# schulter/crbm

Measured on AMD Instinct MI355X. Metric: Gibbs-steps/sec (PCD-1) at batch 8192x4x200, 10 motifs len 15, higher is better.
Workload: dtype f32; 1 GPU; cfg2: 10 motifs len 15, batch 8192 x 4x200, PCD-1, single-stranded; chains_per_gpu=8192, gibbs_steps_per_launch=1, visible=4x200, hidden=10x186, parallelism=chains sharded over 1 GPU(s), no collective in the Gibbs step

## Files before the change

### __graft_entry__.py

```python
import os
import sys

ROOT = os.path.dirname(os.path.abspath(__file__))
if ROOT not in sys.path:
    sys.path.insert(0, ROOT)


PRECOMPILE = [dict(num_motifs=k, motif_length=m, doublestranded=ds) for (k, m, ds) in [
    (10, 15, 0), (10, 15, 1), (50, 25, 0), (20, 15, 1),
    (10, 5, 1), (10, 5, 0), (3, 4, 1), (4, 5, 1), (4, 5, 0), (6, 9, 1), (2, 5, 1),
]]
PRECOMPILE += [dict(num_motifs=6, motif_length=7, doublestranded=1, pooling=2, fantasy_hidden_len=24),
               dict(num_motifs=10, motif_length=15, doublestranded=0, pooling=4, fantasy_hidden_len=48),
               dict(num_motifs=5, motif_length=8, doublestranded=1, pooling=3, fantasy_hidden_len=36)]
PRECOMPILE += [dict(num_motifs=100, motif_length=15, doublestranded=0), dict(num_motifs=20, motif_length=40, doublestranded=1)]
PRECOMPILE += [dict(num_motifs=300, motif_length=10, doublestranded=0, fantasy_hidden_len=51), dict(num_motifs=120, motif_length=40, doublestranded=1, fantasy_hidden_len=61),
               dict(num_motifs=256, motif_length=4, doublestranded=1, fantasy_hidden_len=37), dict(num_motifs=300, motif_length=10, doublestranded=0, batchsize=4096, fantasy_hidden_len=191)]
PRECOMPILE += [dict(num_motifs=300, motif_length=10, doublestranded=0, batchsize=512, fantasy_hidden_len=30),
               dict(num_motifs=120, motif_length=40, doublestranded=1, batchsize=256, fantasy_hidden_len=24)]
PRECOMPILE += [dict(num_motifs=10, motif_length=15, doublestranded=0, batchsize=8192, fantasy_hidden_len=186),
               dict(num_motifs=50, motif_length=25, doublestranded=0, batchsize=8192, fantasy_hidden_len=976),
               dict(num_motifs=20, motif_length=15, doublestranded=1, batchsize=8192, fantasy_hidden_len=486)]
PRECOMPILE += [dict(num_motifs=3, motif_length=3, doublestranded=1, batchsize=4, fantasy_hidden_len=8),
               dict(num_motifs=4, motif_length=4, doublestranded=0, batchsize=4, fantasy_hidden_len=8)]

STATISTICS_SHAPES = [dict(num_motifs=k, motif_length=m, doublestranded=ds, pooling=pool, batchsize=7, fantasy_hidden_len=lf)
                     for (k, m, ds, pool, lf) in [
    (10, 15, 0, 1, 33), (16, 16, 1, 1, 33), (16, 32, 0, 1, 33), (32, 16, 0, 1, 33), (8, 12, 1, 1, 33), (20, 15, 1, 1, 33),
    (33, 17, 0, 1, 33), (64, 32, 1, 1, 33), (20, 40, 1, 1, 33), (4, 64, 1, 1, 33), (100, 15, 0, 1, 33), (130, 7, 1, 1, 33),
    (256, 4, 0, 1, 33), (6, 7, 1, 2, 34), (10, 15, 0, 4, 36), (5, 8, 1, 3, 33), (300, 10, 0, 1, 33), (150, 6, 1, 2, 34),
    (10, 15, 0, 1, 64), (10, 15, 0, 1, 32), (20, 40, 1, 1, 64), (20, 40, 1, 1, 32)]]


def build():
    from crbm_amd.csrc import build as hip_build
    hip_build.build(verbose=True)
    hip_build.prune_cache()
    hip_build.precompile(PRECOMPILE + STATISTICS_SHAPES, verbose=False)
    from oracle import build_cpu
    build_cpu.build(verbose=True)
    import crbm_amd
    from crbm_amd import _lib
    lib = _lib.load()
    assert lib.crbm_abi_version() == _lib.ABI_VERSION
    print("crbm_amd", crbm_amd.__version__, "ABI", lib.crbm_abi_version())


def smoke():
    import numpy as np
    from crbm_amd import CRBM
    from oracle.crbm_oracle import OracleCRBM, synthetic_onehot

    K, M, B, Lf, n, L = 10, 15, 64, 186, 48, 200
    W = np.random.default_rng(42).standard_normal((K, 1, 4, M)).astype(np.float32)
    model = CRBM(K, M, doublestranded=False, batchsize=B, cd_k=1, fantasy_hidden_len=Lf, seed=2026)
    oracle = OracleCRBM(K, M, doublestranded=False, batchsize=B, cd_k=1, fantasy_hidden_len=Lf, seed=2026, W=W)
    b = (oracle.b + 4.0).astype(np.float32)
    model.motifs.set_value(W)
    model.bias.set_value(b)
    oracle.b = b.astype(np.float64)
    D = synthetic_onehot(n, L, seed=1234)
    model._trainingFct(D)
    oracle.train_step(D)
    np.testing.assert_allclose(model.motifs.get_value(), oracle.W, rtol=1e-4, atol=2e-6)
    np.testing.assert_allclose(model.bias.get_value(), oracle.b, rtol=1e-4, atol=2e-6)
    np.testing.assert_allclose(model.c.get_value(), oracle.c, rtol=1e-4, atol=2e-6)
    from oracle.crbm_oracle import hidden_uniforms, visible_uniforms, KIND_CHAIN_H, KIND_CHAIN_V
    model.set_fantasy(oracle.fantasy_h.astype(np.float32))
    idx = np.arange(B) + oracle.seq_offset
    for _ in range(3):
        t = oracle.gibbs_step
        model.set_rng(gibbs_step=t)
        uv = visible_uniforms(oracle.seed, t, idx, Lf + M - 1, KIND_CHAIN_V)
        Pv, v = oracle._computeVgivenH(oracle.fantasy_h, None, uv)
        uh = hidden_uniforms(oracle.seed, t, idx, K, Lf, 0, KIND_CHAIN_H)
        P, hnew = oracle._computeHgivenV(v, False, uh)
        model.gibbsSteps(1)
        h, _ = model.get_fantasy()
        gv = model.get_fantasy_visible()
        badv = (gv != v).any(axis=2)[:, 0]
        if badv.any():
            gap = np.min(np.abs(np.cumsum(Pv[:, 0], axis=1)[:, :3] - uv[:, None, :]), axis=1)
            assert np.all(gap[badv] < 1e-6), "visible sample differs away from a tie"
        bad = (h != hnew) & ~badv.any(axis=1)[:, None, None, None]
        assert np.all(np.abs(P - uh)[bad] < 1e-6), "hidden sample differs away from a tie"
        oracle.fantasy_h, oracle.gibbs_step = hnew, t + 1
        model.set_fantasy(hnew.astype(np.float32))
    assert oracle.fantasy_h.sum() > 0
    np.testing.assert_allclose(model.freeEnergy(D), oracle.freeEnergy(D), rtol=1e-4)
    print("smoke ok: train step, Gibbs chain and free energy match the oracle")


if __name__ == "__main__":
    build()
    if os.path.exists("/dev/kfd"):
        smoke()
```

### crbm_amd/_lib.py

```python
import ctypes
import os

import numpy as np

_HERE = os.path.dirname(os.path.abspath(__file__))
LIB_PATH = os.path.join(_HERE, "csrc", "libcrbm_hip.so")

UNIQUE_ID_BYTES = 128
IPC_HANDLE_BYTES = 64
ABI_VERSION = 5

CRBM_OK = 0
ERR_INVALID, ERR_HIP, ERR_NOT_ONEHOT, ERR_NOT_BINARY, ERR_RCCL, ERR_NO_GPU, ERR_IPC_TIMEOUT = -1, -2, -3, -4, -5, -6, -7


class CrbmConfig(ctypes.Structure):
    _fields_ = [
        ("num_motifs", ctypes.c_int32),
        ("motif_length", ctypes.c_int32),
        ("input_dims", ctypes.c_int32),
        ("doublestranded", ctypes.c_int32),
        ("batchsize", ctypes.c_int32),
        ("cd_k", ctypes.c_int32),
        ("pooling", ctypes.c_int32),
# ... 25 lines not shown
_I32P = ctypes.POINTER(ctypes.c_int32)
_I64P = ctypes.POINTER(ctypes.c_int64)


class CrbmSite(ctypes.Structure):
    _fields_ = [("seq", ctypes.c_int32), ("motif", ctypes.c_int32), ("start", ctypes.c_int32),
                ("strand", ctypes.c_int32), ("prob", ctypes.c_float)]


_SITEP = ctypes.POINTER(CrbmSite)
_SITES_TAIL = [ctypes.c_float, _I64, _SITEP, _I64P, _I32P, _I32P, _F]

SIGNATURES = {
    "crbm_create": (_I32, [ctypes.POINTER(CrbmConfig), ctypes.POINTER(_H)]),
    "crbm_precompile": (_I32, [ctypes.POINTER(CrbmConfig)]),
    "crbm_destroy": (_I32, [_H]),
    "crbm_last_error": (ctypes.c_char_p, [_H]),
    "crbm_abi_version": (_I32, []),
    "crbm_device_count": (_I32, []),
    "crbm_set_params": (_I32, [_H, _F, _F, _F]),
    "crbm_get_params": (_I32, [_H, _F, _F, _F]),
    "crbm_set_velocities": (_I32, [_H, _F, _F, _F]),
    "crbm_get_velocities": (_I32, [_H, _F, _F, _F]),
    "crbm_set_fantasy": (_I32, [_H, _F, _F]),
    "crbm_get_fantasy": (_I32, [_H, _F, _F]),
    "crbm_get_fantasy_visible": (_I32, [_H, _F]),
    "crbm_set_rng": (_I32, [_H, _U64, _U32, _U32]),
    "crbm_get_rng": (_I32, [_H, ctypes.POINTER(_U64), ctypes.POINTER(_U32), ctypes.POINTER(_U32)]),
    "crbm_set_shard": (_I32, [_H, _U32]),
    "crbm_train_step": (_I32, [_H, _F, _I32, _I32]),
    "crbm_dataset_upload": (_I32, [_H, _F, _I32, _I32]),
    "crbm_dataset_upload_codes": (_I32, [_H, _U8P, _I32, _I32]),
    "crbm_dataset_select": (_I32, [_H, _I32]),
    "crbm_train_step_resident": (_I32, [_H, _I32, _I32]),
    "crbm_train_epoch_resident": (_I32, [_H, _I32]),
    "crbm_train_epoch_sharded": (_I32, [_H, _I32, _I32, _I32]),
    "crbm_gibbs_steps": (_I32, [_H, _I32]),
    "crbm_gibbs_steps_async": (_I32, [_H, _I32]),
    "crbm_sync": (_I32, [_H]),
    "crbm_wait_idle": (_I32, [_H]),
    "crbm_time_gibbs": (_I32, [_H, _I32, _I32, _F]),
    "crbm_time_train": (_I32, [_H, _I32, _I32, _I32, _F]),
    "crbm_h_given_v": (_I32, [_H, _F, _I32, _I32, _I32, _U32, _F, _F, _F]),
    "crbm_v_given_h": (_I32, [_H, _F, _F, _I32, _I32, _U32, _F, _F, _F]),
    "crbm_hit_probs": (_I32, [_H, _F, _I32, _I32, _F]),
    "crbm_free_energy": (_I32, [_H, _F, _I32, _I32, _F]),
    "crbm_free_energy_per_motif": (_I32, [_H, _F, _I32, _I32, _F]),
    "crbm_eval_data": (_I32, [_H, _F, _I32, _I32, _F, _F]),
    "crbm_eval_params": (_I32, [_H, _F, _F, _F]),
    "crbm_hit_probs_codes": (_I32, [_H, _U8P, _I32, _I32, _F]),
    "crbm_hit_probs_resident": (_I32, [_H, _I32, _I32, _F]),
    "crbm_free_energy_codes": (_I32, [_H, _U8P, _I32, _I32, _F, _F]),
    "crbm_free_energy_resident": (_I32, [_H, _I32, _I32, _F, _F]),
    "crbm_eval_data_resident": (_I32, [_H, _I32, _I32, _F, _F]),
    "crbm_eval_epoch_resident": (_I32, [_H, _I32, ctypes.POINTER(ctypes.c_double), ctypes.POINTER(ctypes.c_double)]),
    "crbm_hit_summary": (_I32, [_H, _F, _I32, _I32, _F, _F, _F]),
    "crbm_hit_summary_codes": (_I32, [_H, _U8P, _I32, _I32, _F, _F, _F]),
    "crbm_hit_summary_resident": (_I32, [_H, _I32, _I32, _F, _F, _F]),
    "crbm_motif_sites": (_I32, [_H, _F, _I32, _I32] + _SITES_TAIL),
    "crbm_motif_sites_codes": (_I32, [_H, _U8P, _I32, _I32] + _SITES_TAIL),
    "crbm_motif_sites_resident": (_I32, [_H, _I32, _I32] + _SITES_TAIL),
    "crbm_scan_sites_codes": (_I32, [_H, _U8P, _I64, ctypes.c_float, _I64, _SITEP, _I64P]),
    "crbm_scan_histogram_codes": (_I32, [_H, _U8P, _I64, ctypes.c_float, ctypes.c_float, _I32, ctypes.POINTER(_U64), _I64P]),
    "crbm_variant_effects_codes": (_I32, [_H, _U8P, _I64, _I64, _I64P, _U8P, _F, _F, _I32P]),
    "crbm_mutagenesis": (_I32, [_H, _F, _I32, _I32, _F, _F]),
    "crbm_mutagenesis_codes": (_I32, [_H, _U8P, _I32, _I32, _F, _F]),
    "crbm_mutagenesis_resident": (_I32, [_H, _I32, _I32, _F, _F]),
    "crbm_ais": (_I32, [_H, _I32, _I32, _U32, _F, _I32, _I32, _I32, _F, _U64, _U8P, _F]),
    "crbm_comm_unique_id": (_I32, [_U8P]),
    "crbm_comm_init": (_I32, [_H, _U8P, _I32, _I32]),
    "crbm_comm_destroy": (_I32, [_H]),
    "crbm_comm_broadcast_state": (_I32, [_H, _I32]),
    "crbm_ipc_export": (_I32, [_H, _U8P]),
    "crbm_ipc_attach": (_I32, [_H, _U8P, _I32, _I32]),
    "crbm_ipc_detach": (_I32, [_H]),
    "crbm_ipc_status": (_I32, [_H, ctypes.POINTER(_I32)]),
    "crbm_sums_count": (_I32, [_H]),
    "crbm_train_local": (_I32, [_H, _F, _I32, _I32, _F]),
    "crbm_train_apply": (_I32, [_H, _F, _I32]),
    "crbm_time_allreduce": (_I32, [_H, _I32, _F]),
    "crbm_get_launch_info": (_I32, [_H, ctypes.POINTER(CrbmLaunchInfo)]),
    "crbm_copy_bandwidth": (_I32, [_H, ctypes.c_int64, _I32, _F]),
    "crbm_last_shader_clock": (_I32, [_H, _F]),
    "crbm_gibbs_state_bytes": (ctypes.c_int64, [_H]),
}

_lib = None


class CrbmLibraryError(RuntimeError):
    pass


def load():
    global _lib
    if _lib is not None:
        return _lib
    if not os.path.exists(LIB_PATH):
        raise CrbmLibraryError(
            "HIP extension not built: %s is missing. Run `python -m crbm_amd.csrc.build` "
            "(or __graft_entry__.build()). There is no CPU fallback." % LIB_PATH)
    lib = ctypes.CDLL(LIB_PATH)
    for name, (res, args) in SIGNATURES.items():
        fn = getattr(lib, name)
        fn.restype = res
        fn.argtypes = args
    if lib.crbm_abi_version() != ABI_VERSION:
        raise CrbmLibraryError("ABI version mismatch")
    _lib = lib
    return lib


def fptr(arr):
    if arr is None:
        return None
    assert arr.dtype == np.float32 and arr.flags["C_CONTIGUOUS"]
    return arr.ctypes.data_as(_F)


def as_f32(x):
    return np.ascontiguousarray(x, dtype=np.float32)
```

### crbm_amd/csrc/build.py

```python
import os
import subprocess
import sys
from concurrent.futures import ThreadPoolExecutor

HERE = os.path.dirname(os.path.abspath(__file__))
OBJ = os.path.join(HERE, "build")
LIB = os.path.join(HERE, "libcrbm_hip.so")
HIPCC = os.environ.get("HIPCC", "/opt/rocm/bin/hipcc")
ARCH = "gfx950"
FLAGS = ["--offload-arch=" + ARCH, "-O3", "-std=c++17", "-fPIC", "-ffp-contract=off",
         "-Wall", "-Wno-unused-function", "-Wno-unused-result"]
HEADERS = ["crbm_kernels.h", "crbm_kernels_generic.h", "crbm_layout.h", "crbm_jit.h", "crbm_plan.h", "crbm_sweep.h", os.path.join("..", "..", "include", "crbm_amd.h")]


def _newer(target, deps):
    if not os.path.exists(target):
        return True
    t = os.path.getmtime(target)
    return any(os.path.getmtime(d) > t for d in deps)


def _compile(job):
    src, obj, extra = job
    deps = [os.path.join(HERE, src), os.path.abspath(__file__)] + [os.path.join(HERE, h) for h in HEADERS]
    if not _newer(obj, deps):
        return obj, False
    cmd = [HIPCC] + FLAGS + extra + ["-c", os.path.join(HERE, src), "-o", obj]
    r = subprocess.run(cmd, capture_output=True, text=True)
    if r.returncode != 0:
        raise RuntimeError("hipcc failed: %s\n%s\n%s" % (" ".join(cmd), r.stdout, r.stderr))
    if r.stderr.strip():
        sys.stderr.write(r.stderr)
    return obj, True


def build(verbose=True, jobs=None):
    os.makedirs(OBJ, exist_ok=True)
    work = [("crbm_api.hip", os.path.join(OBJ, "crbm_api.o"), [])]
    jobs = jobs or min(8, os.cpu_count() or 4)
    with ThreadPoolExecutor(max_workers=jobs) as ex:
        results = list(ex.map(_compile, work))
    objs = [o for o, _ in results]
    if any(changed for _, changed in results) or _newer(LIB, objs):
        cmd = [HIPCC, "--offload-arch=" + ARCH, "-shared", "-fPIC", "-o", LIB] + objs + ["-L/opt/rocm/lib", "-lhiprtc", "-ldl"]
        r = subprocess.run(cmd, capture_output=True, text=True)
        if r.returncode != 0:
            raise RuntimeError("link failed: %s\n%s\n%s" % (" ".join(cmd), r.stdout, r.stderr))
        if verbose:
            print("built", LIB)
    elif verbose:
        print("up to date:", LIB)
    return LIB


def prune_cache(verbose=True):
    cache = os.path.join(HERE, "jit_cache")
    if not os.path.isdir(cache):
        return 0
    newest = max(os.path.getmtime(os.path.join(HERE, h)) for h in ("crbm_kernels.h", "crbm_layout.h", "crbm_jit.h"))
    gone = 0
    for f in os.listdir(cache):
        path = os.path.join(cache, f)
        if f.endswith((".hsaco", ".tmp")) and os.path.getmtime(path) < newest:
            os.unlink(path)
            gone += 1
    if verbose and gone:
        print("jit cache: removed %d stale code objects" % gone)
    return gone


def precompile(configs, verbose=True):
    import ctypes
    sys.path.insert(0, os.path.dirname(os.path.dirname(HERE)))
    from crbm_amd import _lib
    lib = _lib.load()
    for c in configs:
        cfg = _lib.CrbmConfig(num_motifs=c["num_motifs"], motif_length=c["motif_length"], input_dims=4,
                              doublestranded=int(c.get("doublestranded", 0)), batchsize=c.get("batchsize", 20),
                              cd_k=1, pooling=c.get("pooling", 1), fantasy_hidden_len=c.get("fantasy_hidden_len", 200),
                              learning_rate=0.1, momentum=0.9, rho=0.01, lambda_rate=0.1, seed=0, device=0, reserved=0)
        rc = lib.crbm_precompile(ctypes.byref(cfg))
        if rc != 0:
            raise RuntimeError("precompile failed for %s: %s" % (c, lib.crbm_last_error(None).decode()))
        if verbose:
            print("jit cache ready:", c)


if __name__ == "__main__":
    build()
```

### crbm_amd/csrc/crbm_api.hip

```cpp
#define CRBM_DEFINE_MISC_KERNELS
#include "crbm_kernels.h"
#include "crbm_jit.h"
#include "crbm_plan.h"
#include "crbm_sweep.h"
#include "../../include/crbm_amd.h"

#include <dlfcn.h>
#include <rccl/rccl.h>

#include <algorithm>
#include <chrono>
#include <condition_variable>
#include <deque>
#include <mutex>
#include <thread>
#include <climits>
#include <cmath>
#include <cstdio>
#include <cstdlib>
#include <cstring>
#include <string>
#include <vector>

using namespace crbm;
// ... 91 lines not shown
};

struct crbm_handle {
  crbm_config cfg;
  int K = 0, M = 0, ds = 0, NW = 0, KAM = 0;
  int A = 4;
  int Lf = 0, Lv = 0, B = 0;
  int device = 0, num_cu = 256;
  hipStream_t stream = nullptr;
  hipStream_t stream2 = nullptr;
  hipEvent_t ev0 = nullptr, ev1 = nullptr, ev_fork = nullptr, ev_join = nullptr;
  bool overlap = false;
  LaunchPlan plan;
  bool big() const { return plan.big; }
  const ModelShape& ms() const { return plan.ms; }
  JitKernels jk;
  float* d_tables = nullptr;
  float* d_tf_solo = nullptr;
  bool tables_dirty = true;
  uint64_t params_version = 1, tf_solo_version = 0;
  float *dW = nullptr, *db = nullptr, *dc = nullptr, *dvW = nullptr, *dvb = nullptr, *dvc = nullptr;
  float *dW2 = nullptr, *db2 = nullptr, *dc2 = nullptr, *dvW2 = nullptr, *dvb2 = nullptr, *dvc2 = nullptr;
  uint32_t *d_hm = nullptr, *d_hmp = nullptr, *d_vf = nullptr;
  uint32_t* d_flags = nullptr;
  unsigned long long* d_ones = nullptr;
  DevBuf<float> stage, stage2, out_a, out_b, out_c;
  DevBuf<uint32_t> letters, letters2, masks_tmp;
  DevBuf<float> out_a2, out_b2;
  DevBuf<uint32_t> dataset[CRBM_DATASET_SLOTS];
  DevBuf<float> partials, partials2;
  DevBuf<unsigned long long> eval_ones;
  struct SetBufs {
    DevBuf<SiteRec> site_recs;
    DevBuf<unsigned long long> site_count, site_keys;
    DevBuf<float> mut_df, mut_pll;
    DevBuf<uint32_t> mut_rows;
    DevBuf<unsigned long long> scan_valid, scan_off;
    DevBuf<unsigned short> scan_lanes;
    DevBuf<uint32_t> scan_tiles;
    DevBuf<int32_t> var_windows;
  } set_bufs[2];
  int mut_route = 0;
  DevBuf<float> ais_betas, ais_base, ais_logw;
  DevBuf<uint8_t> ais_state;
  DevBuf<unsigned long long> hist;
  float* d_sums = nullptr;
  int dataset_n[CRBM_DATASET_SLOTS] = {0, 0}, dataset_L[CRBM_DATASET_SLOTS] = {0, 0};
  int slot = 0;
  uint64_t seed = 0;
  uint32_t gibbs_step = 0, eval_step = 0, chain_offset = 0;
  int LWs = 0;
  hipStream_t part_stream[4] = {nullptr, nullptr, nullptr, nullptr};
  PartWorker* part_worker[4] = {nullptr, nullptr, nullptr, nullptr};
  hipEvent_t part_done[4] = {nullptr, nullptr, nullptr, nullptr};
  hipEvent_t ev_parts_fork = nullptr;
  bool forked = false;
  bool main_idle_hint = false;
  double part_launch_us = 0.0;
  hipEvent_t ev_cal0 = nullptr, ev_cal1 = nullptr;
  bool cal_pending = false;
  int wall_khz = 100000;
  int variant = 1;
  int topdown_mode = 0;
  uint32_t* d_nset = nullptr;
  int nset_slots = 0;
  uint32_t launches_since_read = 0;
  double activity = -1.0;
  int stats_rows = 0;
  bool fuse_stats = false;
  bool one_launch = true;
  SumsLayout sl;
  ncclComm_t comm = nullptr;
  int nranks = 1, rank = 0;
  float* ipc_buf = nullptr;
  void* ipc_peer[IPC_MAX_RANKS] = {};
  int ipc_stride = 0;
  bool ipc_on = false;
  uint32_t ipc_step = 0;
  bool ipc_published = false;
  uint32_t* d_ticket = nullptr;
  unsigned long long* d_probe = nullptr;
  unsigned long long probe_base[2] = {0, 0}, probe_last[2] = {0, 0};
  bool probe_on = false;
  unsigned long long* d_timeline = nullptr;
  int timeline_cap = 0, timeline_next = 0;
  unsigned long long ipc_timeout_ticks = 0;
  SlabModel slab;
  float* d_slab_tables = nullptr;
  int slab_n = 0;
  bool slab_hgv = false;
  uint64_t slab_tables_version = 0;
  std::string slab_note;
  std::string err;
};

namespace {

int fail(crbm_handle* h, int code, const std::string& msg) {
  if (h) h->err = msg; else g_create_error = msg;
  return code;
}

#define HIPCHK(expr)                                                                         \
  do {                                                                                       \
    hipError_t e__ = (expr);                                                                 \
    if (e__ != hipSuccess)                                                                   \
      return fail(h, CRBM_ERR_HIP, std::string(#expr) + ": " + hipGetErrorString(e__));      \
  } while (0)

#define ARGCHK(cond, msg)                                 \
  do {                                                    \
    if (!(cond)) return fail(h, CRBM_ERR_INVALID, msg);   \
  } while (0)

RngView rng_view(const crbm_handle* h, uint32_t step, uint32_t seq_offset) {
  RngView r;
  r.seed_lo = (uint32_t)(h->seed & 0xffffffffu);
  r.seed_hi = (uint32_t)(h->seed >> 32);
  r.step = step;
  r.seq_offset = seq_offset;
  return r;
}

int tab_bytes(const ModelShape& ms) { return ms.TAB * 4; }

int lw(const crbm_handle* h, int L) { return letter_words_any(h->A, L); }

int ensure_tables(crbm_handle* h) {
  if (!h->tables_dirty || h->big()) return CRBM_OK;
  TablesArgs t;
  t.W = h->dW; t.b = h->db; t.c = h->dc; t.out = h->d_tables;
  const unsigned grid = (unsigned)std::max(1, std::min((h->ms().TABLES_ALL + 255) / 256, h->num_cu * 4));
  HIPCHK(jit_launch(h->jk.build_tables, t, grid, 1, 256, 0, h->stream));
  h->tables_dirty = false;
  h->main_idle_hint = false;
  return CRBM_OK;
}

int ensure_solo_table(crbm_handle* h) {
  if (h->plan.GS == h->plan.G || h->tf_solo_version == h->params_version) return CRBM_OK;
  TablesArgs t;
  t.W = h->dW; t.b = h->db; t.c = h->dc; t.out = h->d_tf_solo;
  const unsigned grid = (unsigned)std::max(1, std::min((h->plan.ms_solo.TAB + 255) / 256, h->num_cu * 4));
  HIPCHK(jit_launch(h->jk.build_gather_solo, t, grid, 1, 256, 0, h->stream));
  h->tf_solo_version = h->params_version;
  h->main_idle_hint = false;
  return CRBM_OK;
}

BigModel big_model(const crbm_handle* h) {
  BigModel m;
  m.W = h->dW; m.b = h->db; m.c = h->dc;
  m.K = h->K; m.M = h->M; m.ds = h->ds; m.NW = h->NW; m.A = h->A;
  return m;
}

constexpr int SLAB_FALLBACK = -1000;
bool slab_fe_on(const crbm_handle* h) { return h->slab.K && tab_bytes(h->slab.ms) <= 160 * 1024 && env_int("CRBM_SLAB_FE", 1) != 0; }
int slab_launch_hgv(crbm_handle* h, const uint32_t* d_letters, int n, int L, int mode, unsigned long long* ones, uint32_t* masks,
                    uint32_t kind, uint32_t step, uint32_t seq_offset, hipStream_t st);
int slab_launch_stats(crbm_handle* h, const uint32_t* d_letters, int n, int L, bool data_half, hipStream_t st, ReduceArgs* reduce);
int slab_launch_fe(crbm_handle* h, const uint32_t* rows, int n, int L, float* fe, float* fem, DevBuf<float>* scratch, hipStream_t st);

int big_launch_hgv(crbm_handle* h, const uint32_t* d_letters, int n, int L, int mode, float* act, float* prob, float* sample,
                   unsigned long long* ones, uint32_t* masks, uint32_t kind, uint32_t step, uint32_t seq_offset, hipStream_t st) {
  if (h->slab.K && h->slab_hgv && (masks || ones) && !act && !prob && !sample) {
// ... 78 lines not shown
  BigStatsArgs a;
  a.m = big_model(h);
  a.letters = d_letters;
  a.n = n; a.L = L; a.Lh = L - M + 1; a.LW = lw(h, L);
  a.want_sparsity = data_half ? 1 : 0;
  a.R = std::max(1, std::min(n, std::max(1, (h->num_cu * 8) / K)));
  a.pool = h->ms().POOL;
  a.CH = std::max(64, std::min(4096, a.Lh));
  a.CH = std::max(a.pool, a.CH - a.CH % a.pool);
  a.row = 3 * KAM + 3 * K + h->A;
  a.off_vh0 = 0; a.off_vh1 = KAM; a.off_h0 = 2 * KAM; a.off_h1 = 2 * KAM + K;
  a.off_sw = 2 * KAM + 2 * K; a.off_sb = 3 * KAM + 2 * K; a.off_v = 3 * KAM + 3 * K;
  HIPCHK(pbuf.ensure((size_t)a.R * a.row));
  a.partials = pbuf.p;
  ARGCHK(h->A * M <= BIG_ST * 256, "motif_length too large for the statistics kernel");
  const size_t lds = (((size_t)h->A * M + 3) & ~(size_t)3) * 4 + (size_t)(a.pool > 1 ? 5 : 3) * a.CH * 4 + 64 + 12 * 256 * 4 +
                     (size_t)((h->A + 3) & ~3) * 4 + (size_t)a.CH + M;
  ARGCHK(lds <= 160 * 1024, "motif_length too large for the statistics kernel");
  hipLaunchKernelGGL(big_stats_kernel, dim3(K, a.R), dim3(256), lds, st, a);
  HIPCHK(hipGetLastError());
  *reduce = reduce_args(h, data_half, pbuf.p, a.R, a.row, n);
  return CRBM_OK;
}

int big_launch_eval(crbm_handle* h, const uint32_t* rows, int n, int L, int hits, float* fe, float* fem, float* hmax, float* hmean,
                    unsigned long long* pos_fx, DevBuf<float>* fe_scratch, hipStream_t st) {
  if (!hits && slab_fe_on(h)) {
    const int rc = slab_launch_fe(h, rows, n, L, fe, fem, fe_scratch, st);
    if (rc != SLAB_FALLBACK) return rc;
  }
  BigEvalArgs a;
  a.m = big_model(h);
  a.letters = rows;
  a.n = n; a.L = L; a.Lh = L - h->M + 1; a.LW = lw(h, L);
  a.fe = fe; a.fem = fem; a.hmax = hmax; a.hmean = hmean; a.pos_fx = pos_fx; a.hits = hits; a.pool = h->ms().POOL;
  const size_t lds = (((size_t)h->A * h->M + 3) & ~(size_t)3) * 4 + 64 + (size_t)L;
  ARGCHK(lds <= 160 * 1024, "sequence too long for the evaluation kernel of a model of this size");
  hipLaunchKernelGGL(big_eval_kernel, dim3(std::max(1, std::min(n, h->num_cu * 8))), dim3(256), lds, st, a);
  HIPCHK(hipGetLastError());
  return CRBM_OK;
}

int grid_for(long items, int threads, int cap) {
  long g = (items + threads - 1) / threads;
  return (int)std::max<long>(1, std::min<long>(g, cap));
}

int tile_seqs(int len, int target) { return std::max(1, std::min(target / std::max(1, len), (1 << 20) / std::max(1, len))); }

int check_flags(crbm_handle* h) {
  uint32_t flags = 0;
  HIPCHK(hipMemcpyAsync(&flags, h->d_flags, sizeof(flags), hipMemcpyDeviceToHost, h->stream));
  HIPCHK(hipStreamSynchronize(h->stream));
  if (flags) {
    HIPCHK(hipMemsetAsync(h->d_flags, 0, sizeof(uint32_t), h->stream));
    if (flags & 1u) return fail(h, CRBM_ERR_NOT_ONEHOT, "visible data is not exactly one-hot");
    return fail(h, CRBM_ERR_NOT_BINARY, "hidden state is not exactly 0/1");
  }
  return CRBM_OK;
}

int launch_hgv(crbm_handle* h, const uint32_t* d_letters, int n, int L, int mode, float* act, float* prob,
               float* sample, unsigned long long* ones, uint32_t kind, uint32_t step, uint32_t seq_offset) {
  if (h->big()) return big_launch_hgv(h, d_letters, n, L, mode, act, prob, sample, ones, nullptr, kind, step, seq_offset, h->stream);
  int rc = ensure_tables(h);
  if (rc) return rc;
  HgvArgs a;
  a.tables = h->d_tables;
  a.letters = d_letters;
  a.n = n; a.L = L; a.Lh = L - h->M + 1; a.LW = lw(h, L);
  a.TS = tile_seqs(a.Lh, 4096);
  a.divLh = make_fastdiv((uint32_t)a.Lh);
  a.mode = mode;
  a.act = act; a.prob = prob; a.sample = sample; a.ones = ones;
  a.rng = rng_view(h, step, seq_offset);
  a.kind = kind;
  const int ntiles = (n + a.TS - 1) / a.TS;
  const unsigned gx = (unsigned)std::max(1, std::min(ntiles, h->num_cu * 8));
  HIPCHK(jit_launch(h->jk.hgv, a, gx, 1, 256, (unsigned)tab_bytes(h->ms()), h->stream));
  return CRBM_OK;
}

StatsGeom stats_geom(const StatsMfmaLayout& st, float* partials, long ngroups, int lds_bytes);

int prepare_gibbs(crbm_handle* h, const ChainGeom& g, int steps, ReduceArgs* model_reduce, GibbsArgs* out, unsigned* lds_out) {
  const GibbsLayout& gl = g.gl;
  GibbsArgs& a = *out;
  a.tables = h->d_tables;
  a.tables_tf = nullptr; a.off_ws = 0;
  a.hm = h->d_hm; a.hmp = h->ds ? h->d_hmp : nullptr; a.vout = h->d_vf;
  a.nchains = h->B; a.Lf = h->Lf; a.Lv = gl.Lv; a.S = gl.S;
  a.nvb = gl.nvb; a.nhb = gl.nhb; a.Lrow = gl.Lrow; a.LWs = gl.LWs;
  a.divVB = make_fastdiv((uint32_t)a.nvb);
  a.divHB = make_fastdiv((uint32_t)a.nhb);
  a.divRow = make_fastdiv((uint32_t)(a.Lrow * h->NW));
  a.divLfw = make_fastdiv((uint32_t)(a.Lf * h->NW));
  a.steps = steps;
  a.rng = rng_view(h, h->gibbs_step, h->chain_offset);
  a.ones = h->d_nset;
  a.clock = h->probe_on ? h->d_probe : nullptr;
  a.timeline = nullptr;
  a.debug = env_int("CRBM_GIBBS_DEBUG", 0);
  a.nblocks = g.grid;
  a.stats_off = 0;
  a.sg = StatsGeom();
  unsigned lds = (unsigned)gl.lds_bytes;
  if (model_reduce) {
    const StatsMfmaLayout st = stats_mfma_layout(h->ms(), 0, h->Lf, g.threads, 0, false);
    HIPCHK(h->partials2.ensure((size_t)g.grid * st.row));
    a.stats_off = (gl.lds_bytes / 4 + 3) & ~3;
    lds = (unsigned)std::max((a.stats_off + st.region_floats) * 4, st.combine_bytes);
    a.sg = stats_geom(st, h->partials2.p, (long)gl.S * st.GPC, (int)lds);
    *model_reduce = reduce_args(h, false, h->partials2.p, g.grid, st.row, h->B);
  }
  *lds_out = lds;
  return CRBM_OK;
}

void part_worker_main(PartWorker* w) {
  (void)hipSetDevice(w->device);
  std::unique_lock<std::mutex> lock(w->mu);
  for (;;) {
    const auto spin_until_t = std::chrono::steady_clock::now() + std::chrono::milliseconds(2);
    while (!w->stop && w->jobs.empty() && std::chrono::steady_clock::now() < spin_until_t) {
      lock.unlock();
      for (int i = 0; i < 64; ++i) __builtin_ia32_pause();
      lock.lock();
    }
    w->cv.wait(lock, [&] { return w->stop || !w->jobs.empty(); });
    if (w->jobs.empty()) return;
    PartJob job = w->jobs.front();
    w->jobs.pop_front();
    w->busy = true;
    lock.unlock();
    hipError_t e = hipSuccess;
    if (job.delay_ticks > 0) {
      hipLaunchKernelGGL(delay_kernel, dim3(1), dim3(64), 0, w->stream, job.delay_ticks);
      e = hipGetLastError();
    }
    if (e == hipSuccess) e = jit_launch(job.fn, job.args, job.grid, 1, job.threads, job.lds, w->stream);
    lock.lock();
    if (e != hipSuccess && w->error == hipSuccess) w->error = e;
    w->busy = false;
    if (w->jobs.empty()) w->idle_cv.notify_all();
  }
}

int drain_part_workers(crbm_handle* h) {
  for (int p = 1; p < h->plan.chain_parts; ++p) {
    PartWorker* w = h->part_worker[p];
    if (!w) continue;
    std::unique_lock<std::mutex> lock(w->mu);
    w->idle_cv.wait(lock, [&] { return w->jobs.empty() && !w->busy; });
    if (w->error != hipSuccess) {
      const hipError_t e = w->error;
      w->error = hipSuccess;
      return fail(h, CRBM_ERR_HIP, std::string("chain launch of partition ") + std::to_string(p) + ": " + hipGetErrorString(e));
    }
  }
  return CRBM_OK;
}

int join_parts(crbm_handle* h) {
  if (!h->forked) return CRBM_OK;
  {
    const int rc = drain_part_workers(h);
    if (rc) return rc;
  }
  for (int p = 1; p < h->plan.chain_parts; ++p) {
    HIPCHK(hipEventRecord(h->part_done[p], h->part_stream[p]));
    HIPCHK(hipStreamWaitEvent(h->stream, h->part_done[p], 0));
  }
  h->forked = false;
  return CRBM_OK;
}

int launch_gibbs_parts(crbm_handle* h, int steps) {
  bool first_of_fork = false;
  double stagger_ticks = 0.0;
  if (!h->forked) {
    if (!h->main_idle_hint && hipStreamQuery(h->stream) != hipSuccess) {
      (void)hipGetLastError();
      HIPCHK(hipEventRecord(h->ev_parts_fork, h->stream));
      for (int p = 1; p < h->plan.chain_parts; ++p) HIPCHK(hipStreamWaitEvent(h->part_stream[p], h->ev_parts_fork, 0));
    }
    h->main_idle_hint = false;
    h->forked = true;
    first_of_fork = true;
    if (h->cal_pending && hipEventQuery(h->ev_cal1) == hipSuccess) {
      float ms = 0.f;
      if (hipEventElapsedTime(&ms, h->ev_cal0, h->ev_cal1) == hipSuccess && ms > 0.f) h->part_launch_us = 1e3 * ms;
      h->cal_pending = false;
    }
    (void)hipGetLastError();
    if (env_int("CRBM_PART_STAGGER", 1)) {
      const double est = h->part_launch_us > 0.0 ? h->part_launch_us
                                                 : 1e-3 * (double)h->B * h->Lf * h->K * (1 + h->ds) * steps;
      stagger_ticks = 0.9 * est / h->plan.chain_parts * (h->wall_khz / 1000.0);
    }
  }
  const LaunchPlan& plan = h->plan;
  GibbsArgs a;
  unsigned lds = 0;
  const int rc = prepare_gibbs(h, plan.part, steps, nullptr, &a, &lds);
  if (rc) return rc;
  const unsigned grid = (unsigned)plan.part.grid, threads = (unsigned)plan.part.threads;
  const size_t per = (size_t)h->Lf * h->NW;
  const int waves = (int)threads / 64;
  h->nset_slots = plan.chain_parts * (int)grid * waves;
  for (int p = 0; p < plan.chain_parts; ++p) {
    const int c0 = p * plan.part_chains, n = std::min(plan.part_chains, h->B - c0);
    if (n <= 0) break;
    GibbsArgs ap = a;
    ap.hm = a.hm + (size_t)c0 * per;
    if (ap.hmp) ap.hmp = a.hmp + (size_t)c0 * per;
    ap.vout = a.vout + (size_t)c0 * a.LWs;
    ap.nchains = n;
    ap.rng.seq_offset = a.rng.seq_offset + (uint32_t)c0;
    ap.ones = a.ones + (size_t)p * grid * waves;
    if (p > 0) ap.clock = nullptr;
    if (h->d_timeline && h->timeline_next < h->timeline_cap) ap.timeline = h->d_timeline + 2 * (size_t)(h->timeline_next++);
    ap.nblocks = (int)grid;
    if (p > 0) {
      PartWorker* w = h->part_worker[p];
      {
        std::lock_guard<std::mutex> lock(w->mu);
        w->jobs.push_back(PartJob{h->jk.gibbs_sparse, ap, grid, threads, lds, (unsigned long long)(stagger_ticks * p)});
      }
      w->cv.notify_one();
      continue;
    }
    const bool calibrate = first_of_fork && !h->cal_pending;
    if (calibrate) HIPCHK(hipEventRecord(h->ev_cal0, h->part_stream[0]));
    HIPCHK(jit_launch(h->jk.gibbs_sparse, ap, grid, 1, threads, lds, h->part_stream[0]));
    if (calibrate) {
      HIPCHK(hipEventRecord(h->ev_cal1, h->part_stream[0]));
      h->cal_pending = true;
    }
  }
  h->gibbs_step += (uint32_t)steps;
  h->launches_since_read += 1;
  return CRBM_OK;
}

int launch_gibbs(crbm_handle* h, int steps, hipStream_t s = nullptr, ReduceArgs* model_reduce = nullptr, bool plain = false) {
  if (!s) s = h->stream;
  if (h->big()) return big_launch_gibbs(h, steps, s);
  int rc = ensure_tables(h);
  if (rc) return rc;
  if (plain && !model_reduce && h->variant == 1 && h->plan.chain_parts > 1 && s == h->stream) return launch_gibbs_parts(h, steps);
  const ChainGeom& g = model_reduce ? h->plan.chain[h->variant] : plain_geom(h->plan, h->variant, false);
  GibbsArgs a;
  unsigned lds = 0;
  rc = prepare_gibbs(h, g, steps, model_reduce, &a, &lds);
  if (!model_reduce && h->variant == 1 && h->plan.GS != h->plan.G) {
    a.tables_tf = h->d_tf_solo; a.off_ws = h->ms().OFF_WS;
    if (rc == CRBM_OK) rc = ensure_solo_table(h);
  }
  if (rc) return rc;
  h->nset_slots = g.grid * (g.threads / 64);
  if (plain && h->d_timeline && h->timeline_next < h->timeline_cap) a.timeline = h->d_timeline + 2 * (size_t)(h->timeline_next++);
  hipFunction_t fn = model_reduce ? h->jk.gibbs_sparse_stats : (h->variant ? h->jk.gibbs_sparse : h->jk.gibbs);
  HIPCHK(jit_launch(fn, a, (unsigned)g.grid, 1, (unsigned)g.threads, lds, s));
  h->gibbs_step += (uint32_t)steps;
  h->launches_since_read += 1;
  return CRBM_OK;
}

int refresh_activity(crbm_handle* h) {
  if (h->launches_since_read == 0) return CRBM_OK;
  if (h->big()) {
    unsigned long long on = 0;
    HIPCHK(hipMemcpy(&on, h->d_ones, sizeof(on), hipMemcpyDeviceToHost));
    h->launches_since_read = 0;
    h->activity = (double)on / ((double)h->B * h->Lf * h->K * (1 + h->ds));
    return CRBM_OK;
  }
  std::vector<uint32_t> slots((size_t)h->nset_slots);
  HIPCHK(hipMemcpy(slots.data(), h->d_nset, slots.size() * sizeof(uint32_t), hipMemcpyDeviceToHost));
  unsigned long long last = 0;
  for (uint32_t v : slots) last += v;
  h->launches_since_read = 0;
  h->activity = (double)last / ((double)h->B * h->Lf * h->K * (1 + h->ds));
  return CRBM_OK;
}

StatsGeom stats_geom(const StatsMfmaLayout& st, float* partials, long ngroups, int lds_bytes) {
  StatsGeom g;
  g.GPC = st.GPC;
  g.lds_floats = lds_bytes / 4;
  g.off_slices = st.off_slices; g.slice = st.slice;
  g.off_win = st.off_win; g.off_gw = st.off_gw; g.off_pt = st.off_pt;
  g.divGPC = make_fastdiv((uint32_t)st.GPC, (uint64_t)std::max<long>(ngroups, 1));
  g.row = st.row; g.off_vh0 = st.off_vh[0]; g.off_vh1 = st.off_vh[1]; g.off_h0 = st.off_h[0]; g.off_h1 = st.off_h[1];
  g.off_sw = st.off_sw; g.off_sb = st.off_sb; g.off_v = st.off_v;
  g.partials = partials;
  return g;
}

struct StatsLaunch { int lds = 0, grid = 0, block = 0, row = 0; };
int prepare_stats(crbm_handle* h, const ModelShape& ms, const float* tables, DevBuf<float>& pbuf, const uint32_t* d_letters, int n, int L,
                  bool data_half, int threads, StatsMfmaArgs* out, StatsLaunch* launch) {
  const int want_sp = data_half ? 1 : 0;
  const int Lh = L - ms.M + 1;
  const int tabs = tab_bytes(ms);
  const bool own = threads <= 0;
  const StatsMfmaLayout st = stats_mfma_layout(ms, want_sp, Lh, own ? env_int("CRBM_STATS_THREADS", 0) : threads, tabs, own,
                                               env_int("CRBM_STATS_MAX_TILES", CRBM_STATS_MAX_TILES));
  StatsMfmaArgs& a = *out;
  a.tables = tables;
  a.letters = d_letters;
  a.n = n; a.L = L; a.Lh = Lh; a.LW = lw(h, L);
  const long ngroups = (long)n * st.GPC;
  const long nunits = (ngroups + 1) / 2;
  a.off_tab = st.region_floats;
  a.debug = env_int("CRBM_STATS_DEBUG", 0);
  ARGCHK(ngroups < (1L << 31), "batch too large for the statistics kernel");
  const int lds = std::max(st.region_floats * 4 + tabs, st.combine_bytes);
  ARGCHK(lds <= 160 * 1024, "model too large for the statistics kernel");
  const int wpr = (st.threads / 64) / st.NR;
  const int per_cu = own ? std::max(1, std::min(2048 / st.threads, (160 * 1024) / std::max(1, lds))) : 3;
  const long cap = h->stats_rows > 0 ? h->stats_rows : own ? (long)h->num_cu * per_cu : std::max<long>(1, (long)h->num_cu * 3 * 256 / st.threads);
  const long upw = std::max<long>(1, (nunits + cap * wpr - 1) / (cap * wpr));
  const int gx = (int)std::max<long>(1, (nunits + upw * wpr - 1) / (upw * wpr));
  HIPCHK(pbuf.ensure((size_t)gx * st.row));
  a.nblocks = gx;
  a.sg = stats_geom(st, pbuf.p, ngroups, lds);
  launch->lds = lds; launch->grid = gx; launch->block = st.threads; launch->row = st.row;
  return CRBM_OK;
}

int slab_origin(const crbm_handle* h, int i) {
  const int Ks = h->slab.K;
  if ((i + 1) * Ks <= h->K) return i * Ks;
  return h->slab_hgv ? ((h->K - Ks + 9) / 10) * 10 : h->K - Ks;
}

SlabPlan slab_plan(const crbm_handle* h) {
  SlabPlan p;
  p.Ks = h->slab.K; p.K = h->K; p.last_k0 = slab_origin(h, h->slab_n - 1);
  return p;
}

int slab_ensure_tables(crbm_handle* h, hipStream_t st) {
  const SlabModel* s = &h->slab;
// ... 180 lines not shown
  h->params_version += 1;
}

int launch_update(crbm_handle* h, int L_data) {
  UpdateTablesArgs a;
  fill_update_args(h, L_data, a);
  if (h->big()) {
    UpdateArgs& u = a.u;
    u.oW = h->dW; u.ob = h->db; u.oc = h->dc; u.ovW = h->dvW; u.ovb = h->dvb; u.ovc = h->dvc;
    hipLaunchKernelGGL(big_update_kernel, dim3(grid_for((long)h->KAM + h->K + h->A, 256, h->num_cu * 4)), dim3(256), 0, h->stream, u);
    HIPCHK(hipGetLastError());
    h->params_version += 1;
    return CRBM_OK;
  }
  const unsigned grid = (unsigned)std::max(1, std::min((h->ms().TABLES_ALL + 4095) / 4096, 32));
  HIPCHK(jit_launch(h->jk.update_tables, a, grid, 1, UPDATE_THREADS, (unsigned)((h->KAM + h->K + 4) * 4), h->stream));
  swap_param_sets(h);
  return CRBM_OK;
}

size_t ipc_bytes(const crbm_handle* h);
float* ipc_slot_of(void* base, const crbm_handle* h, int parity, int source);
uint32_t* ipc_flag_of(void* base, const crbm_handle* h, int parity, int source);

int launch_reduce_pair(crbm_handle* h, ReducePair pair, bool publish) {
  if (pair.half[0].row == 0 || pair.half[1].row == 0) {
    for (auto& half : pair.half)
      if (half.row > 0) {
        hipLaunchKernelGGL(reduce_partials_kernel, dim3((half.row + 31) / 32), dim3(1024), 0, h->stream, half);
        HIPCHK(hipGetLastError());
      }
    return CRBM_OK;
  }
  const dim3 grid((pair.half[0].row + 31) / 32, 2);
  if (publish && h->ipc_on) {
    const int parity = (int)(h->ipc_step & 1u);
    float* base = ipc_slot_of(h->ipc_buf, h, parity, h->rank);
    for (auto& half : pair.half) half.sums = base + (half.sums - h->d_sums);
    PublishTail t;
    t.ticket = h->d_ticket; t.value = h->ipc_step + 1u;
    t.push.n = h->nranks;
    for (int r = 0; r < IPC_MAX_RANKS; ++r) {
      void* peer = r < h->nranks ? h->ipc_peer[r] : h->ipc_buf;
      t.push.delta[r] = (long long)(reinterpret_cast<char*>(ipc_slot_of(peer, h, parity, h->rank)) - reinterpret_cast<char*>(base));
      t.flag[r] = ipc_flag_of(peer, h, parity, h->rank);
    }
    hipLaunchKernelGGL(reduce_publish_pair_kernel, grid, dim3(1024), 0, h->stream, pair, t);
    h->ipc_published = true;
  } else {
    hipLaunchKernelGGL(reduce_partials_pair_kernel, grid, dim3(1024), 0, h->stream, pair);
  }
  HIPCHK(hipGetLastError());
  return CRBM_OK;
}

int train_local_dev(crbm_handle* h, const uint32_t* d_letters, int n, int L, bool publish = false) {
  int rc = ensure_tables(h);
  if (rc) return rc;
  if (h->slab.K) {
    rc = slab_ensure_tables(h, h->stream);
    if (rc) return rc;
  }
  hipStream_t sm = h->overlap ? h->stream2 : h->stream;
  if (h->overlap) {
    HIPCHK(hipEventRecord(h->ev_fork, h->stream));
    HIPCHK(hipStreamWaitEvent(h->stream2, h->ev_fork, 0));
  }
  ReducePair pair;
  const bool paired = !h->overlap && n > 0;
  if (h->fuse_stats && paired && h->one_launch) {
    const ChainGeom& g = h->plan.chain[h->variant];
    TrainLocalArgs t;
    unsigned glds = 0;
    rc = prepare_gibbs(h, g, h->cfg.cd_k, &pair.half[1], &t.g, &glds);
    if (rc) return rc;
    StatsLaunch d;
    rc = prepare_stats(h, h->ms(), h->d_tables, h->partials, d_letters, n, L, true, g.threads, &t.d, &d);
    if (rc) return rc;
    pair.half[0] = reduce_args(h, true, h->partials.p, d.grid, d.row, n);
    const unsigned lds = std::max(glds, (unsigned)d.lds);
    t.g.sg.lds_floats = (int)(lds / 4);
    t.d.sg.lds_floats = (int)(lds / 4);
    h->nset_slots = g.grid * (g.threads / 64);
    HIPCHK(jit_launch(h->jk.train_local, t, (unsigned)(g.grid + d.grid), 1, (unsigned)g.threads, lds, h->stream));
    h->gibbs_step += (uint32_t)h->cfg.cd_k;
    h->launches_since_read += 1;
    return launch_reduce_pair(h, pair, publish);
  }
  if (h->fuse_stats) {
    ReduceArgs mr;
    rc = launch_gibbs(h, h->cfg.cd_k, sm, &mr);
    if (rc) return rc;
    if (paired) pair.half[1] = mr;
    else {
      hipLaunchKernelGGL(reduce_partials_kernel, dim3((mr.row + 31) / 32), dim3(1024), 0, sm, mr);
      HIPCHK(hipGetLastError());
    }
  } else {
    rc = launch_gibbs(h, h->cfg.cd_k, sm);
    if (rc) return rc;
    rc = join_parts(h);
    if (rc) return rc;
    rc = launch_stats(h, h->d_vf, h->B, h->Lv, false, sm, paired ? &pair.half[1] : nullptr);
    if (rc) return rc;
  }
  if (h->overlap) HIPCHK(hipEventRecord(h->ev_join, h->stream2));
  if (n > 0) {
    rc = launch_stats(h, d_letters, n, L, true, nullptr, paired ? &pair.half[0] : nullptr);
    if (rc) return rc;
    if (paired) {
      rc = launch_reduce_pair(h, pair, publish);
      if (rc) return rc;
    }
  } else {
    HIPCHK(hipMemsetAsync(h->d_sums + h->sl.data_off, 0, (size_t)(h->sl.n_d + 1 - h->sl.data_off) * sizeof(float), h->stream));
  }
  if (h->overlap) HIPCHK(hipStreamWaitEvent(h->stream, h->ev_join, 0));
  return CRBM_OK;
}

size_t ipc_bytes(const crbm_handle* h) { return ((size_t)2 * IPC_MAX_RANKS * h->ipc_stride + (2 * IPC_MAX_RANKS + 1) * 16) * sizeof(float); }
float* ipc_slot_of(void* base, const crbm_handle* h, int parity, int source) {
  return static_cast<float*>(base) + ((size_t)parity * IPC_MAX_RANKS + source) * h->ipc_stride;
}
uint32_t* ipc_flag_of(void* base, const crbm_handle* h, int parity, int source) {
  return reinterpret_cast<uint32_t*>(static_cast<float*>(base) + (size_t)2 * IPC_MAX_RANKS * h->ipc_stride) + 16 * (parity * IPC_MAX_RANKS + source);
}
uint32_t* ipc_status_of(void* base, const crbm_handle* h) {
  return reinterpret_cast<uint32_t*>(static_cast<float*>(base) + (size_t)2 * IPC_MAX_RANKS * h->ipc_stride) + 16 * 2 * IPC_MAX_RANKS;
}

int ipc_allocate(crbm_handle* h) {
  if (h->ipc_buf) return CRBM_OK;
  h->ipc_stride = (h->sl.count + 31) & ~31;
  void* p = nullptr;
  const hipError_t fe = hipExtMallocWithFlags(&p, ipc_bytes(h), hipDeviceMallocFinegrained);
  if (fe != hipSuccess) {
    (void)hipGetLastError();
    if (env_int("CRBM_IPC_COARSE_OK", 0) == 0)
      return fail(h, CRBM_ERR_HIP, std::string("hipExtMallocWithFlags(hipDeviceMallocFinegrained) for the mapped sums buffer: ") + hipGetErrorString(fe));
    HIPCHK(hipMalloc(&p, ipc_bytes(h)));
  }
  HIPCHK(hipMemset(p, 0, ipc_bytes(h)));
  h->ipc_buf = static_cast<float*>(p);
  return CRBM_OK;
}

int launch_ipc_allreduce_update(crbm_handle* h, int L_data) {
  const int parity = (int)(h->ipc_step & 1u);
  const uint32_t value = h->ipc_step + 1u;
  if (!h->ipc_published) {
    PublishArgs pa;
    pa.src = h->d_sums; pa.value = value; pa.count = h->sl.count; pa.n = h->nranks;
    for (int r = 0; r < IPC_MAX_RANKS; ++r) {
      void* peer = r < h->nranks ? h->ipc_peer[r] : h->ipc_buf;
      pa.dst[r] = ipc_slot_of(peer, h, parity, h->rank);
      pa.flag[r] = ipc_flag_of(peer, h, parity, h->rank);
    }
    hipLaunchKernelGGL(publish_sums_kernel, dim3(1), dim3(1024), 0, h->stream, pa);
    HIPCHK(hipGetLastError());
  }
  h->ipc_published = false;
  UpdateIpcArgs a;
  fill_update_args(h, L_data, a.ut);
  for (int r = 0; r < IPC_MAX_RANKS; ++r) {
    const int src = r < h->nranks ? r : 0;
    a.ipc.sums[r] = ipc_slot_of(h->ipc_buf, h, parity, src);
// ... 246 lines not shown
        HIPCHK(hipStreamSynchronize(set.st));
        if (timing) {
          float ms = 0.f;
          HIPCHK(hipEventElapsedTime(&ms, tev[si][0], tev[si][1]));
          device_ms += ms;
          ++segments;
        }
        return CRBM_OK;
      },
      [&] { sweep_drain(h); });
    if (rc) return rc;
    if (timing) fprintf(stderr, "%s: kernels %.3f ms over %d segments\n", api, device_ms, segments);
    HIPCHK(hipStreamSynchronize(h->stream2));
    HIPCHK(hipStreamSynchronize(h->stream));
    uint32_t flags = 0;
    HIPCHK(hipMemcpyAsync(&flags, h->d_flags, sizeof(flags), hipMemcpyDeviceToHost, h->stream));
    HIPCHK(hipStreamSynchronize(h->stream));
    if (flags) {
      HIPCHK(hipMemsetAsync(h->d_flags, 0, sizeof(uint32_t), h->stream));
      HIPCHK(hipStreamSynchronize(h->stream));
      return fail(h, CRBM_ERR_INVALID, "stream codes must lie in 0..4 (0..3 = A,C,G,T; 4 = no letter)");
    }
    return CRBM_OK;
  }
};

}

extern "C" {

int crbm_abi_version(void) { return CRBM_AMD_ABI_VERSION; }

int crbm_device_count(void) {
  int n = 0;
  if (hipGetDeviceCount(&n) != hipSuccess) return 0;
  return n;
}

const char* crbm_last_error(const crbm_handle* h) { return h ? h->err.c_str() : g_create_error.c_str(); }

}

namespace {

int validate_config(const crbm_config* cfg) {
  crbm_handle* h = nullptr;
  if (!cfg) return fail(h, CRBM_ERR_INVALID, "null argument");
  ARGCHK(cfg->num_motifs >= 1, "Number of motifs must be positive.");
  ARGCHK(cfg->num_motifs <= 65536, "num_motifs > 65536 is not supported");
  ARGCHK(cfg->motif_length >= 1, "Motif length must be positive.");
  ARGCHK(cfg->input_dims >= 1, "input_dims must be positive.");
  ARGCHK(cfg->input_dims <= 64, "input_dims > 64 is not supported (v|h keeps a position's activations of all letters in LDS)");
  ARGCHK(cfg->input_dims * cfg->motif_length <= 256 * BIG_ST, "input_dims * motif_length > 2048 is not supported (statistics kernel: one accumulator per letter and filter column, 8 per thread of a 256-thread block; DNA: motif_length <= 512)");
  ARGCHK((long)cfg->num_motifs * cfg->motif_length * cfg->input_dims <= (1L << 26), "num_motifs * input_dims * motif_length too large");
  ARGCHK(cfg->pooling >= 1 && cfg->pooling <= 64, "pooling must be between 1 and 64");
  ARGCHK(cfg->fantasy_hidden_len % cfg->pooling == 0, "pooling must divide the hidden length of the fantasy chains");
  ARGCHK(cfg->batchsize >= 1, "batchsize must be positive.");
  ARGCHK(cfg->cd_k >= 1, "cd_k must be positive.");
  ARGCHK(cfg->fantasy_hidden_len >= 1 && cfg->fantasy_hidden_len <= 65536, "fantasy_hidden_len out of range");
  ARGCHK(cfg->rho > 0.f && cfg->rho < 1.f, "rho must be in (0,1)");
  ARGCHK(cfg->learning_rate > 0.f, "learning_rate must be positive.");
  ARGCHK(cfg->momentum >= 0.f && cfg->momentum < 1.f, "momentum must be between zero and one.");
  ARGCHK(cfg->lambda_rate >= 0.f, "lambda_rate must be non-negative.");
  return CRBM_OK;
}

}

extern "C" {

int crbm_precompile(const crbm_config* cfg) {
  int rc = validate_config(cfg);
  if (rc) return rc;
  const LaunchPlan p = plan_launches(cfg->num_motifs, cfg->motif_length, cfg->doublestranded ? 1 : 0, cfg->input_dims, cfg->pooling,
                                     cfg->fantasy_hidden_len > 0 ? cfg->fantasy_hidden_len : 200, cfg->batchsize, env_int("CRBM_NUM_CU", 256));
  std::vector<char> code;
  bool cached = false;
  std::string file, err;
  int rc_jit = 0;
  if (!p.big)
    rc_jit = jit_compile(p.ms.K, p.ms.M, p.ms.DS, p.G, p.GS, p.ms.POOL, p.gibbs_wpe, p.gibbs_tb, &code, &cached, &file, &err);
  else if (p.slab_K > 0)
    rc_jit = jit_compile(p.slab_K, p.ms.M, p.ms.DS, p.slab_G, p.slab_G, p.slab_ms.POOL, 0, 256, &code, &cached, &file, &err, true);
  if (rc_jit != 0) {
    g_create_error = err;
    return CRBM_ERR_HIP;
  }
  return CRBM_OK;
}

int crbm_create(const crbm_config* cfg, crbm_handle** out) {
  crbm_handle* h = nullptr;
  if (!cfg || !out) return fail(h, CRBM_ERR_INVALID, "null argument");
  *out = nullptr;
  int rc = validate_config(cfg);
  if (rc) return rc;
  int ndev = 0;
  if (hipGetDeviceCount(&ndev) != hipSuccess || ndev <= 0)
    return fail(h, CRBM_ERR_NO_GPU, "no HIP device visible (this library has no CPU path)");
  ARGCHK(cfg->device >= 0 && cfg->device < ndev, "device ordinal out of range");

  crbm_handle* hh = new crbm_handle();
  hh->cfg = *cfg;
  hh->K = cfg->num_motifs; hh->M = cfg->motif_length; hh->ds = cfg->doublestranded ? 1 : 0;
  hh->A = cfg->input_dims;
  hh->KAM = hh->K * hh->A * hh->M;
  hh->Lf = cfg->fantasy_hidden_len; hh->Lv = hh->Lf + hh->M - 1; hh->B = cfg->batchsize;
  hh->seed = cfg->seed;
  hh->device = cfg->device;
  hh->sl = sums_layout(hh->K, hh->M, hh->A);
  auto bail = [&](int code) { crbm_destroy(hh); return code; };
  hipError_t e;
#define TRY(expr)                                                                                 \
  if ((e = (expr)) != hipSuccess) {                                                               \
    g_create_error = std::string(#expr) + ": " + hipGetErrorString(e);                            \
    return bail(CRBM_ERR_HIP);                                                                    \
  }
  TRY(hipSetDevice(hh->device));
  hipDeviceProp_t prop;
  TRY(hipGetDeviceProperties(&prop, hh->device));
  hh->num_cu = prop.multiProcessorCount > 0 ? prop.multiProcessorCount : 256;
  {
    int khz = 0;
    if (hipDeviceGetAttribute(&khz, hipDeviceAttributeWallClockRate, hh->device) == hipSuccess && khz > 0) hh->wall_khz = khz;
    (void)hipGetLastError();
  }
  hh->plan = plan_launches(hh->K, hh->M, hh->ds, hh->A, cfg->pooling, hh->Lf, hh->B, hh->num_cu);
  const LaunchPlan& plan = hh->plan;
  hh->NW = plan.ms.NW;
  if (plan.refusal) {
    g_create_error = plan.refusal;
    return bail(CRBM_ERR_INVALID);
  }
  hh->LWs = hh->big() ? letter_words_any(hh->A, hh->Lv) : plan.chain[1].gl.LWs;
  hh->variant = 1; hh->topdown_mode = 2;
  if (!hh->big()) {
    const char* td = getenv("CRBM_TOPDOWN");
    hh->topdown_mode = (td && !strcmp(td, "dense") && plan.has_dense) ? 1 : 2;
    hh->variant = hh->topdown_mode == 1 ? 0 : 1;
    std::string err;
    if (jit_load(hh->K, hh->M, hh->ds, plan.G, plan.GS, hh->ms().POOL, plan.gibbs_wpe, plan.gibbs_tb, &hh->jk, &err) != 0) {
      g_create_error = "kernel specialisation failed: " + err;
      return bail(CRBM_ERR_HIP);
    }
  }
  TRY(hipStreamCreateWithFlags(&hh->stream, hipStreamNonBlocking));
  TRY(hipStreamCreateWithFlags(&hh->stream2, hipStreamNonBlocking));
  TRY(hipEventCreate(&hh->ev0));
  TRY(hipEventCreate(&hh->ev1));
  TRY(hipEventCreateWithFlags(&hh->ev_fork, hipEventDisableTiming));
  TRY(hipEventCreateWithFlags(&hh->ev_join, hipEventDisableTiming));
  if (plan.chain_parts > 1) {
    TRY(hipEventCreateWithFlags(&hh->ev_parts_fork, hipEventDisableTiming));
    TRY(hipEventCreate(&hh->ev_cal0));
    TRY(hipEventCreate(&hh->ev_cal1));
    hh->part_stream[0] = hh->stream;
    for (int p = 1; p < plan.chain_parts; ++p) {
      TRY(hipStreamCreateWithFlags(&hh->part_stream[p], hipStreamNonBlocking));
      TRY(hipEventCreate(&hh->part_done[p]));
      {
        PartWorker* w = new PartWorker();
        w->device = hh->device;
        w->stream = hh->part_stream[p];
        w->th = std::thread(part_worker_main, w);
        hh->part_worker[p] = w;
      }
    }
  }
  hh->overlap = env_int("CRBM_OVERLAP", 0) != 0;
  const size_t pad_k = hh->big() ? 10 : 0;
  const size_t kam = (size_t)hh->KAM + pad_k * hh->A * hh->M, k = (size_t)hh->K + pad_k;
  TRY(hipMalloc((void**)&hh->dW, kam * 4)); TRY(hipMalloc((void**)&hh->dvW, kam * 4));
  TRY(hipMalloc((void**)&hh->db, k * 4));   TRY(hipMalloc((void**)&hh->dvb, k * 4));
  const size_t cb = (size_t)std::max(4, hh->A) * 4;
  TRY(hipMalloc((void**)&hh->dc, cb));      TRY(hipMalloc((void**)&hh->dvc, cb));
  TRY(hipMemset(hh->dW, 0, kam * 4)); TRY(hipMemset(hh->dvW, 0, kam * 4));
  TRY(hipMemset(hh->db, 0, k * 4));   TRY(hipMemset(hh->dvb, 0, k * 4));
  TRY(hipMemset(hh->dc, 0, cb));      TRY(hipMemset(hh->dvc, 0, cb));
  TRY(hipMalloc((void**)&hh->dW2, kam * 4)); TRY(hipMalloc((void**)&hh->dvW2, kam * 4));
  TRY(hipMalloc((void**)&hh->db2, k * 4));   TRY(hipMalloc((void**)&hh->dvb2, k * 4));
  TRY(hipMalloc((void**)&hh->dc2, cb));      TRY(hipMalloc((void**)&hh->dvc2, cb));
  TRY(hipMalloc((void**)&hh->d_tables, hh->big() ? 64 : (size_t)hh->ms().TABLES_ALL * 4));
  if (plan.GS != plan.G) TRY(hipMalloc((void**)&hh->d_tf_solo, (size_t)plan.ms_solo.TAB * 4));
  const size_t mwords = (size_t)hh->B * hh->Lf * hh->NW;
  TRY(hipMalloc((void**)&hh->d_hm, mwords * 4)); TRY(hipMemset(hh->d_hm, 0, mwords * 4));
  TRY(hipMalloc((void**)&hh->d_hmp, mwords * 4)); TRY(hipMemset(hh->d_hmp, 0, mwords * 4));
  const size_t vwords = (size_t)hh->B * hh->LWs;
  TRY(hipMalloc((void**)&hh->d_vf, vwords * 4)); TRY(hipMemset(hh->d_vf, 0, vwords * 4));
  TRY(hipMalloc((void**)&hh->d_flags, 16)); TRY(hipMemset(hh->d_flags, 0, 16));
  TRY(hipMalloc((void**)&hh->d_ones, 16)); TRY(hipMemset(hh->d_ones, 0, 16));
  {
    size_t slots = plan.part.on() ? (size_t)plan.chain_parts * plan.part.grid * (plan.part.threads / 64) : 0;
    for (const ChainGeom* g : {&plan.chain[0], &plan.chain[1], &plan.solo})
      if (g->on()) slots = std::max(slots, (size_t)g->grid * (g->threads / 64));
    slots += 64;
    TRY(hipMalloc((void**)&hh->d_nset, slots * 4)); TRY(hipMemset(hh->d_nset, 0, slots * 4));
  }
  TRY(hipMalloc((void**)&hh->d_sums, (size_t)hh->sl.count * 4)); TRY(hipMemset(hh->d_sums, 0, (size_t)hh->sl.count * 4));
  TRY(hipMalloc((void**)&hh->d_ticket, 16)); TRY(hipMemset(hh->d_ticket, 0, 16));
  TRY(hipMalloc((void**)&hh->d_probe, 32)); TRY(hipMemset(hh->d_probe, 0, 32));
  TRY(hipDeviceSynchronize());
#undef TRY
  hh->tables_dirty = true;
  {
    const char* sv = getenv("CRBM_STATS");
    hh->fuse_stats = !hh->big() && hh->ms().FUSE_STATS && hh->variant == 1 && !(sv && !strcmp(sv, "split"));
    hh->one_launch = !(sv && !strcmp(sv, "two"));
    if (hh->fuse_stats) {
      const ChainGeom& g = plan.chain[hh->variant];
      const StatsMfmaLayout st = stats_mfma_layout(hh->ms(), 0, hh->Lf, g.threads, 0, false);
      const int lds = std::max((((g.gl.lds_bytes / 4 + 3) & ~3) + st.region_floats) * 4, st.combine_bytes);
      if (lds > 160 * 1024) hh->fuse_stats = false;
    }
  }
  hh->stats_rows = env_int("CRBM_STATS_ROWS", 0);
  slab_setup(hh);
  *out = hh;
  return CRBM_OK;
}

int crbm_destroy(crbm_handle* h) {
  if (!h) return CRBM_OK;
  (void)hipSetDevice(h->device);
  if (h->stream) (void)hipStreamSynchronize(h->stream);
  if (h->stream2) (void)hipStreamSynchronize(h->stream2);
  for (int p = 0; p < 4; ++p) {
    if (PartWorker* w = h->part_worker[p]) {
      {
        std::lock_guard<std::mutex> lock(w->mu);
        w->stop = true;
      }
      w->cv.notify_one();
      if (w->th.joinable()) w->th.join();
      delete w;
      h->part_worker[p] = nullptr;
    }
    if (p > 0 && h->part_stream[p]) { (void)hipStreamSynchronize(h->part_stream[p]); (void)hipStreamDestroy(h->part_stream[p]); }
    if (h->part_done[p]) (void)hipEventDestroy(h->part_done[p]);
  }
  if (h->ev_parts_fork) (void)hipEventDestroy(h->ev_parts_fork);
  if (h->ev_cal0) (void)hipEventDestroy(h->ev_cal0);
  if (h->ev_cal1) (void)hipEventDestroy(h->ev_cal1);
  if (h->comm && g_rccl.CommDestroy) g_rccl.CommDestroy(h->comm);
  for (int r = 0; r < IPC_MAX_RANKS; ++r)
    if (h->ipc_peer[r] && h->ipc_peer[r] != h->ipc_buf) (void)hipIpcCloseMemHandle(h->ipc_peer[r]);
  if (h->ipc_buf) (void)hipFree(h->ipc_buf);
  slab_destroy(h);
  void* ptrs[] = {h->dW2, h->db2, h->dc2, h->dvW2, h->dvb2, h->dvc2, h->dW, h->db, h->dc, h->dvW, h->dvb, h->dvc, h->d_hm, h->d_hmp, h->d_vf, h->d_flags, h->d_ones, h->d_nset, h->d_sums, h->d_ticket, h->d_tables, h->d_tf_solo, h->d_probe, h->d_timeline};
  for (void* p : ptrs)
    if (p) (void)hipFree(p);
  h->stage.release(); h->stage2.release(); h->out_a.release(); h->out_b.release(); h->out_c.release();
  h->letters.release(); h->letters2.release(); h->masks_tmp.release(); h->out_a2.release(); h->out_b2.release();
  for (auto& d : h->dataset) d.release(); h->partials.release(); h->partials2.release();
  for (auto& b : h->set_bufs) {
    b.site_recs.release(); b.site_count.release(); b.site_keys.release();
    b.scan_valid.release(); b.scan_off.release(); b.scan_lanes.release(); b.scan_tiles.release();
    b.mut_df.release(); b.mut_pll.release(); b.mut_rows.release(); b.var_windows.release();
  }
  h->ais_betas.release(); h->ais_base.release(); h->ais_logw.release(); h->ais_state.release(); h->hist.release();
  if (h->jk.module) (void)hipModuleUnload(h->jk.module);
  if (h->ev0) (void)hipEventDestroy(h->ev0);
  if (h->ev1) (void)hipEventDestroy(h->ev1);
  if (h->ev_fork) (void)hipEventDestroy(h->ev_fork);
  if (h->ev_join) (void)hipEventDestroy(h->ev_join);
  if (h->stream2) (void)hipStreamDestroy(h->stream2);
  if (h->stream) (void)hipStreamDestroy(h->stream);
  delete h;
  return CRBM_OK;
}

#define ENTER_ASYNC()                                         \
  if (!h) return CRBM_ERR_INVALID;                            \
  h->err.clear();                                             \
  HIPCHK(hipSetDevice(h->device))
#define ENTER()                                               \
  ENTER_ASYNC();                                              \
  do {                                                        \
    const int jrc__ = join_parts(h);                          \
    if (jrc__) return jrc__;                                  \
  } while (0)

int crbm_set_params(crbm_handle* h, const float* W, const float* b, const float* c) {
  ENTER();
  ARGCHK(W && b && c, "null argument");
  HIPCHK(hipMemcpyAsync(h->dW, W, (size_t)h->KAM * 4, hipMemcpyHostToDevice, h->stream));
  HIPCHK(hipMemcpyAsync(h->db, b, (size_t)h->K * 4, hipMemcpyHostToDevice, h->stream));
  HIPCHK(hipMemcpyAsync(h->dc, c, (size_t)h->A * 4, hipMemcpyHostToDevice, h->stream));
  HIPCHK(hipStreamSynchronize(h->stream));
  h->tables_dirty = true;
  h->params_version += 1;
  return CRBM_OK;
}

int crbm_get_params(crbm_handle* h, float* W, float* b, float* c) {
  ENTER();
  ARGCHK(W && b && c, "null argument");
  HIPCHK(hipMemcpyAsync(W, h->dW, (size_t)h->KAM * 4, hipMemcpyDeviceToHost, h->stream));
  HIPCHK(hipMemcpyAsync(b, h->db, (size_t)h->K * 4, hipMemcpyDeviceToHost, h->stream));
  HIPCHK(hipMemcpyAsync(c, h->dc, (size_t)h->A * 4, hipMemcpyDeviceToHost, h->stream));
  HIPCHK(hipStreamSynchronize(h->stream));
  return CRBM_OK;
}

int crbm_set_velocities(crbm_handle* h, const float* vW, const float* vb, const float* vc) {
  ENTER();
  ARGCHK(vW && vb && vc, "null argument");
  HIPCHK(hipMemcpyAsync(h->dvW, vW, (size_t)h->KAM * 4, hipMemcpyHostToDevice, h->stream));
  HIPCHK(hipMemcpyAsync(h->dvb, vb, (size_t)h->K * 4, hipMemcpyHostToDevice, h->stream));
  HIPCHK(hipMemcpyAsync(h->dvc, vc, (size_t)h->A * 4, hipMemcpyHostToDevice, h->stream));
  HIPCHK(hipStreamSynchronize(h->stream));
  return CRBM_OK;
}

int crbm_get_velocities(crbm_handle* h, float* vW, float* vb, float* vc) {
  ENTER();
  ARGCHK(vW && vb && vc, "null argument");
  HIPCHK(hipMemcpyAsync(vW, h->dvW, (size_t)h->KAM * 4, hipMemcpyDeviceToHost, h->stream));
  HIPCHK(hipMemcpyAsync(vb, h->dvb, (size_t)h->K * 4, hipMemcpyDeviceToHost, h->stream));
  HIPCHK(hipMemcpyAsync(vc, h->dvc, (size_t)h->A * 4, hipMemcpyDeviceToHost, h->stream));
  HIPCHK(hipStreamSynchronize(h->stream));
  return CRBM_OK;
}

int crbm_set_fantasy(crbm_handle* h, const float* hid, const float* hid_prime) {
  ENTER();
  ARGCHK(hid, "null argument");
  ARGCHK(!h->ds || hid_prime, "doublestranded model needs hid_prime");
  const size_t count = (size_t)h->B * h->K * h->Lf;
  HIPCHK(h->stage.ensure(count));
  const float* src[2] = {hid, hid_prime};
  uint32_t* dst[2] = {h->d_hm, h->d_hmp};
  for (int sidx = 0; sidx < 1 + h->ds; ++sidx) {
    HIPCHK(hipMemcpyAsync(h->stage.p, src[sidx], count * 4, hipMemcpyHostToDevice, h->stream));
    HiddenPackArgs a;
    a.dense = h->stage.p; a.masks = dst[sidx]; a.flags = h->d_flags;
    a.n = h->B; a.K = h->K; a.Lh = h->Lf; a.NW = h->NW;
    hipLaunchKernelGGL(pack_hidden_kernel, dim3(grid_for((long)h->B * h->Lf, 256, h->num_cu * 8)), dim3(256), 0, h->stream, a);
    HIPCHK(hipGetLastError());
    HIPCHK(hipStreamSynchronize(h->stream));
  }
  return check_flags(h);
}

// ... 1412 lines not shown
  if (rc) return rc;
  HIPCHK(hipStreamSynchronize(h->stream));
  return CRBM_OK;
}

int crbm_train_apply(crbm_handle* h, const float* sums_in, int32_t L_data) {
  ENTER();
  ARGCHK(sums_in && L_data >= h->M, "bad argument");
  HIPCHK(hipMemcpyAsync(h->d_sums, sums_in, (size_t)h->sl.count * 4, hipMemcpyHostToDevice, h->stream));
  int rc = launch_update(h, L_data);
  if (rc) return rc;
  HIPCHK(hipStreamSynchronize(h->stream));
  return CRBM_OK;
}

int crbm_time_allreduce(crbm_handle* h, int32_t launches, float* total_ms) {
  ENTER();
  ARGCHK(launches >= 1 && total_ms, "bad argument");
  *total_ms = 0.f;
  if (!h->comm) return CRBM_OK;
  HIPCHK(hipEventRecord(h->ev0, h->stream));
  for (int i = 0; i < launches; ++i) {
    ncclResult_t r = g_rccl.AllReduce(h->d_sums, h->d_sums, (size_t)h->sl.count, ncclFloat, ncclSum, h->comm, h->stream);
    if (r != ncclSuccess) return fail(h, CRBM_ERR_RCCL, std::string("ncclAllReduce: ") + g_rccl.GetErrorString(r));
  }
  HIPCHK(hipEventRecord(h->ev1, h->stream));
  HIPCHK(spin_until(h->ev1));
  HIPCHK(hipEventElapsedTime(total_ms, h->ev0, h->ev1));
  return CRBM_OK;
}

int crbm_get_launch_info(const crbm_handle* h, crbm_launch_info* out) {
  if (!h || !out) return CRBM_ERR_INVALID;
  if (h->big()) {
    *out = crbm_launch_info();
    out->gibbs_sparse = 1; out->chain_parts = 1; out->gibbs_block = 256;
    out->activity_ppm = h->activity < 0.0 ? -1 : (int32_t)(h->activity * 1e6 + 0.5);
    out->mutagenesis_route = h->mut_route;
    return CRBM_OK;
  }
  const int tabs = h->ms().TAB * 4;
  const StatsMfmaLayout st = stats_mfma_layout(h->ms(), 1, h->Lf, 0, tabs);
  const int lds = std::max(st.region_floats * 4 + tabs, st.combine_bytes);
  const ChainGeom& g = plain_geom(h->plan, h->variant);
  out->nq = h->ms().NQ; out->group = h->plan.GS;
  out->chain_parts = h->variant == 1 ? h->plan.chain_parts : 1;
  out->gibbs_grid = g.grid; out->gibbs_block = g.threads;
  out->gibbs_seqs_per_tile = g.gl.S; out->gibbs_lds_bytes = g.gl.lds_bytes;
  out->stats_grid_x = h->stats_rows > 0 ? h->stats_rows
                                        : h->num_cu * std::max(1, std::min(2048 / st.threads, (160 * 1024) / std::max(1, lds)));
  out->stats_grid_y = 1;
  out->stats_block = st.threads; out->stats_lds_bytes = lds;
  out->stats_fused = h->fuse_stats ? 1 : 0;
  out->gibbs_sparse = h->variant;
  out->activity_ppm = h->activity < 0.0 ? -1 : (int32_t)(h->activity * 1e6 + 0.5);
  out->mutagenesis_route = h->mut_route;
  return CRBM_OK;
}

int crbm_copy_bandwidth(crbm_handle* h, int64_t bytes, int32_t reps, float* gb_per_s) {
  ENTER();
  ARGCHK(bytes >= (1 << 20) && reps >= 1 && gb_per_s, "bad argument");
  const size_t n4 = (size_t)bytes / 16;
  float4 *src = nullptr, *dst = nullptr;
  HIPCHK(hipMalloc((void**)&src, n4 * 16));
  hipError_t e = hipMalloc((void**)&dst, n4 * 16);
  if (e != hipSuccess) { (void)hipFree(src); return fail(h, CRBM_ERR_HIP, "hipMalloc (copy buffer)"); }
  (void)hipMemsetAsync(src, 1, n4 * 16, h->stream);
  const unsigned grid = (unsigned)((n4 + 1023) / 1024);
  for (int i = 0; i < 1 + reps; ++i) {
    if (i == 1) (void)hipEventRecord(h->ev0, h->stream);
    hipLaunchKernelGGL(copy_float4_kernel, dim3(grid), dim3(256), 0, h->stream, src, dst, n4);
  }
  (void)hipEventRecord(h->ev1, h->stream);
  e = hipEventSynchronize(h->ev1);
  float ms = 0.f;
  if (e == hipSuccess) e = hipEventElapsedTime(&ms, h->ev0, h->ev1);
  (void)hipFree(src); (void)hipFree(dst);
  if (e != hipSuccess) return fail(h, CRBM_ERR_HIP, std::string("copy bandwidth: ") + hipGetErrorString(e));
  *gb_per_s = (float)(2.0 * (double)n4 * 16.0 * reps / (ms * 1e-3) / 1e9);
  return CRBM_OK;
}

int crbm_last_shader_clock(crbm_handle* h, float* mhz) {
  ENTER();
  ARGCHK(mhz, "null argument");
  *mhz = 0.f;
  HIPCHK(hipStreamSynchronize(h->stream));
  HIPCHK(hipMemcpy(h->probe_last, h->d_probe, sizeof(h->probe_last), hipMemcpyDeviceToHost));
  const unsigned long long ticks = h->probe_last[0] - h->probe_base[0], cycles = h->probe_last[1] - h->probe_base[1];
  if (ticks) *mhz = (float)((double)cycles / ((double)ticks / (h->wall_khz / 1000.0)));
  return CRBM_OK;
}

int64_t crbm_gibbs_state_bytes(const crbm_handle* h) {
  if (!h) return 0;
  const int64_t masks = (int64_t)h->B * h->Lf * h->NW * 4 * (1 + h->ds);
  const int64_t vout = (int64_t)h->B * h->LWs * 4;
  return 2 * masks + vout;
}

}
```

### crbm_amd/csrc/crbm_jit.h

```cpp
#pragma once
#include <dlfcn.h>
#include <hip/hip_runtime.h>
#include <hip/hiprtc.h>
#include <sys/stat.h>
#include <unistd.h>

#include <cstdio>
#include <cstdlib>
#include <fstream>
#include <sstream>
#include <mutex>
#include <string>
#include <unordered_map>
#include <vector>

namespace crbm {

struct JitKernels {
  hipModule_t module = nullptr;
  hipFunction_t build_tables = nullptr, update_tables = nullptr, update_tables_ipc = nullptr, hgv = nullptr, gibbs = nullptr ,
                build_gather_solo = nullptr , slab_hgv = nullptr, slab_tables = nullptr, slab_stats_data = nullptr, slab_stats_model = nullptr, slab_fe = nullptr ,
                gibbs_sparse = nullptr, gibbs_sparse_stats = nullptr , train_local = nullptr , stats_mfma_data = nullptr, stats_mfma_model = nullptr,
                free_energy = nullptr, hit_summary = nullptr, motif_sites = nullptr, mutagenesis = nullptr , ais = nullptr , scan_sites = nullptr , scan_hist = nullptr , variant_effects = nullptr ;
  bool from_cache = false;
  std::string cache_file;
};

inline std::string jit_dirname(const std::string& p) {
  const size_t pos = p.find_last_of('/');
  return pos == std::string::npos ? std::string(".") : p.substr(0, pos);
}

inline std::string jit_source_dir() {
  if (const char* e = getenv("CRBM_KERNEL_SRC_DIR")) return e;
  Dl_info info;
  if (dladdr(reinterpret_cast<const void*>(&jit_source_dir), &info) && info.dli_fname) return jit_dirname(info.dli_fname);
  return ".";
}

inline bool jit_read_file(const std::string& path, std::string* out) {
  std::ifstream f(path, std::ios::binary);
  if (!f) return false;
  std::ostringstream ss;
  ss << f.rdbuf();
  *out = ss.str();
  return true;
}

inline uint64_t jit_fnv1a(const std::string& s, uint64_t h = 1469598103934665603ull) {
  for (unsigned char ch : s) {
    h ^= ch;
    h *= 1099511628211ull;
  }
  return h;
}

inline std::string jit_stub(int K, int M, int DS, int G, int GS, int POOL, int gibbs_wpe, int gibbs_tb = 256, bool slab = false) {
  char attr[96] = "", sattr[96] = "";
  if (gibbs_wpe > 0) snprintf(attr, sizeof(attr), "__attribute__((amdgpu_waves_per_eu(1, %d)))", gibbs_wpe);
  else snprintf(attr, sizeof(attr), "__attribute__((amdgpu_waves_per_eu(4)))");
  if (gibbs_wpe > 0) snprintf(sattr, sizeof(sattr), "__attribute__((amdgpu_waves_per_eu(1, %d)))", gibbs_wpe);
  else snprintf(sattr, sizeof(sattr), "__attribute__((amdgpu_waves_per_eu(4)))");
  char buf[24576];
  const int len = snprintf(buf, sizeof(buf),
           "#define CRBM_SLAB_KERNELS %d\n"
           "#include \"crbm_kernels.h\"\n"
           "#ifndef CRBM_GIBBS_ATTR\n#define CRBM_GIBBS_ATTR %s\n#endif\n"
           "#ifndef CRBM_GIBBS_STATS_ATTR\n#define CRBM_GIBBS_STATS_ATTR %s\n#endif\n"
           "#ifndef CRBM_STATS_BYTE_LUT\n#define CRBM_STATS_BYTE_LUT true\n#endif\n"
           "#ifndef CRBM_FUSED_TB\n#define CRBM_FUSED_TB 256\n#endif\n"
           "using ModelCfg = crbm::Cfg<%d, %d, %d, %d, %d>;\n"
           "using SoloCfg = crbm::Cfg<%d, %d, %d, %d, %d>;\n"
           "extern \"C\" __global__ void __launch_bounds__(256) crbm_build_tables(crbm::TablesArgs a) { crbm::build_tables_body<ModelCfg>(a); }\n"
           "extern \"C\" __global__ void __launch_bounds__(256) crbm_build_gather_solo(crbm::TablesArgs a) { crbm::build_gather_table_body<SoloCfg>(a); }\n"
           "extern \"C\" __global__ void __launch_bounds__(1024) crbm_update_tables(crbm::UpdateTablesArgs a) { crbm::update_tables_body<ModelCfg>(a); }\n"
           "extern \"C\" __global__ void __launch_bounds__(1024) crbm_update_tables_ipc(crbm::UpdateIpcArgs a) { crbm::update_tables_ipc_body<ModelCfg>(a); }\n"
           "extern \"C\" __global__ void __launch_bounds__(256) crbm_hgv(crbm::HgvArgs a) { crbm::hgv_body<ModelCfg>(a); }\n"
           "extern \"C\" __global__ void __launch_bounds__(256) crbm_slab_hgv(crbm::SlabHgvArgs a) { if constexpr (CRBM_SLAB_KERNELS && ModelCfg::K <= 64) crbm::slab_hgv_body<ModelCfg>(a); }\n"
           "extern \"C\" __global__ void __launch_bounds__(256) crbm_slab_tables(crbm::SlabTablesArgs a) { if constexpr (CRBM_SLAB_KERNELS && ModelCfg::K <= 64) crbm::slab_tables_body<ModelCfg>(a); }\n"
           "extern \"C\" __global__ void __launch_bounds__(%d) CRBM_GIBBS_ATTR crbm_gibbs_sparse(crbm::GibbsArgs a) { crbm::gibbs_body<SoloCfg, true>(a); }\n"
           "extern \"C\" __global__ void __launch_bounds__(CRBM_FUSED_TB) CRBM_GIBBS_STATS_ATTR crbm_gibbs_sparse_stats(crbm::GibbsArgs a) { if constexpr (ModelCfg::FUSE_STATS) crbm::gibbs_body<ModelCfg, true, true>(a); }\n"
           "extern \"C\" __global__ void __launch_bounds__(CRBM_FUSED_TB) CRBM_GIBBS_STATS_ATTR crbm_train_local(crbm::TrainLocalArgs a) { crbm::train_local_body<ModelCfg>(a); }\n"
           "extern \"C\" __global__ void __launch_bounds__(%d) crbm_gibbs(crbm::GibbsArgs a) { if constexpr (ModelCfg::DENSE) crbm::gibbs_body<ModelCfg, ModelCfg::DENSE ? false : true>(a); }\n"
           "using RoleData = crbm::StatsRole<ModelCfg, true>;\nusing RoleModel = crbm::StatsRole<ModelCfg, false>;\n"
           "extern \"C\" __global__ void __launch_bounds__(RoleData::THREADS) crbm_stats_mfma_data(crbm::StatsMfmaArgs a) { crbm::stats_mfma_body<ModelCfg, true, CRBM_STATS_BYTE_LUT>(a); }\n"
           "extern \"C\" __global__ void __launch_bounds__(RoleModel::THREADS) crbm_stats_mfma_model(crbm::StatsMfmaArgs a) { crbm::stats_mfma_body<ModelCfg, false, CRBM_STATS_BYTE_LUT>(a); }\n"
           "extern \"C\" __global__ void __launch_bounds__(RoleData::THREADS) crbm_slab_stats_data(crbm::SlabStatsArgs a) { if constexpr (CRBM_SLAB_KERNELS && ModelCfg::K <= 64) crbm::slab_stats_body<ModelCfg, true, CRBM_STATS_BYTE_LUT>(a); }\n"
           "extern \"C\" __global__ void __launch_bounds__(RoleModel::THREADS) crbm_slab_stats_model(crbm::SlabStatsArgs a) { if constexpr (CRBM_SLAB_KERNELS && ModelCfg::K <= 64) crbm::slab_stats_body<ModelCfg, false, CRBM_STATS_BYTE_LUT>(a); }\n"
           "extern \"C\" __global__ void __launch_bounds__(256) crbm_free_energy(crbm::FeArgs a) { crbm::free_energy_body<ModelCfg>(a); }\n"
           "extern \"C\" __global__ void __launch_bounds__(256) crbm_slab_fe(crbm::SlabFeArgs a) { if constexpr (CRBM_SLAB_KERNELS && ModelCfg::K <= 64) crbm::slab_fe_body<ModelCfg>(a); }\n"
           "extern \"C\" __global__ void __launch_bounds__(256) crbm_hit_summary(crbm::HitArgs a) { crbm::hit_summary_body<ModelCfg>(a); }\n"
           "extern \"C\" __global__ void __launch_bounds__(256) crbm_motif_sites(crbm::SitesArgs a) { crbm::motif_sites_body<ModelCfg>(a); }\n"
           "extern \"C\" __global__ void __launch_bounds__(256) crbm_mutagenesis(crbm::MutArgs a) { crbm::mutagenesis_body<ModelCfg>(a); }\n"
           "extern \"C\" __global__ void __launch_bounds__(256) crbm_ais(crbm::AisArgs a) { crbm::ais_body<ModelCfg>(a); }\n"
           "extern \"C\" __global__ void __launch_bounds__(256) crbm_scan_sites(crbm::ScanArgs a) { crbm::scan_sites_body<ModelCfg>(a); }\n"
           "extern \"C\" __global__ void __launch_bounds__(512) crbm_scan_hist(crbm::ScanHistArgs a) { crbm::scan_hist_body<ModelCfg>(a); }\n"
           "extern \"C\" __global__ void __launch_bounds__(256) crbm_variant_effects(crbm::VariantArgs a) { crbm::variant_effects_body<ModelCfg>(a); }\n",
           slab ? 1 : 0, attr, sattr, K, M, DS, G, POOL, K, M, DS, GS, POOL, gibbs_tb, gibbs_tb);
  if (len < 0 || len >= (int)sizeof(buf)) return std::string("#error \"jit_stub: the stub outgrew its buffer\"\n");
  return buf;
}

inline int jit_compile(int K, int M, int DS, int G, int GS, int POOL, int gibbs_wpe, int gibbs_tb, std::vector<char>* code, bool* from_cache,
                       std::string* cache_file, std::string* err, bool slab = false) {
  const std::string dir = jit_source_dir();
  std::string kernels, layout;
  if (!jit_read_file(dir + "/crbm_kernels.h", &kernels) || !jit_read_file(dir + "/crbm_layout.h", &layout)) {
    *err = "kernel sources not found in " + dir + " (set CRBM_KERNEL_SRC_DIR)";
    return -1;
  }
  const std::string stub = jit_stub(K, M, DS, G, GS, POOL, gibbs_wpe, gibbs_tb, slab);
  std::vector<std::string> opts = {"--offload-arch=gfx950", "-O3", "-std=c++17", "-ffp-contract=off",
                                   "-I" + dir, "-I/opt/rocm/include"};
  if (const char* e = getenv("CRBM_JIT_DEFINES")) {
    std::istringstream ss(e);
    std::string tok;
    while (ss >> tok) opts.push_back(tok);
  }
  int rtc_major = 0, rtc_minor = 0;
  hiprtcVersion(&rtc_major, &rtc_minor);
  uint64_t h = jit_fnv1a(stub);
  h = jit_fnv1a(kernels, h);
  h = jit_fnv1a(layout, h);
  for (const auto& o : opts)
    if (o.rfind("-I", 0) != 0) h = jit_fnv1a(o, h);
  h = jit_fnv1a(std::to_string(rtc_major) + "." + std::to_string(rtc_minor), h);
  std::string cdir = dir + "/jit_cache";
  if (const char* e = getenv("CRBM_JIT_CACHE")) cdir = e;
  char name[64];
  snprintf(name, sizeof(name), "/crbm_%016llx.hsaco", (unsigned long long)h);
  const std::string cfile = cdir + name;
  if (cache_file) *cache_file = cfile;
  std::string cached;
  if (!getenv("CRBM_JIT_NOCACHE") && jit_read_file(cfile, &cached) && cached.size() > 64) {
    code->assign(cached.begin(), cached.end());
    *from_cache = true;
    return 0;
  }
  *from_cache = false;
  hiprtcProgram prog = nullptr;
  if (hiprtcCreateProgram(&prog, stub.c_str(), "crbm_model.hip", 0, nullptr, nullptr) != HIPRTC_SUCCESS) {
    *err = "hiprtcCreateProgram failed";
    return -1;
  }
  std::vector<const char*> copts;
  for (const auto& o : opts) copts.push_back(o.c_str());
  const hiprtcResult r = hiprtcCompileProgram(prog, (int)copts.size(), copts.data());
  if (r != HIPRTC_SUCCESS) {
    size_t ls = 0;
    hiprtcGetProgramLogSize(prog, &ls);
    std::string log(ls, '\0');
    if (ls) hiprtcGetProgramLog(prog, &log[0]);
    *err = std::string("hiprtc: ") + hiprtcGetErrorString(r) + "\n" + log;
    hiprtcDestroyProgram(&prog);
    return -1;
  }
  size_t cs = 0;
  hiprtcGetCodeSize(prog, &cs);
  code->resize(cs);
  hiprtcGetCode(prog, code->data());
  hiprtcDestroyProgram(&prog);
  mkdir(cdir.c_str(), 0755);
  const std::string tmp = cfile + "." + std::to_string((long)getpid()) + ".tmp";
  {
    std::ofstream f(tmp, std::ios::binary);
    if (f) {
      f.write(code->data(), (std::streamsize)code->size());
      f.close();
      if (rename(tmp.c_str(), cfile.c_str()) != 0) unlink(tmp.c_str());
    }
  }
  return 0;
}

inline int jit_load(int K, int M, int DS, int G, int GS, int POOL, int gibbs_wpe, int gibbs_tb, JitKernels* out, std::string* err, bool slab = false) {
  std::vector<char> code;
  if (jit_compile(K, M, DS, G, GS, POOL, gibbs_wpe, gibbs_tb, &code, &out->from_cache, &out->cache_file, err, slab) != 0) return -1;
  hipError_t e = hipModuleLoadData(&out->module, code.data());
  if (e != hipSuccess) {
    *err = std::string("hipModuleLoadData: ") + hipGetErrorString(e);
    return -1;
  }
  struct { const char* name; hipFunction_t* f; } syms[] = {
      {"crbm_build_tables", &out->build_tables}, {"crbm_build_gather_solo", &out->build_gather_solo}, {"crbm_update_tables", &out->update_tables}, {"crbm_update_tables_ipc", &out->update_tables_ipc}, {"crbm_hgv", &out->hgv}, {"crbm_slab_hgv", &out->slab_hgv}, {"crbm_slab_tables", &out->slab_tables}, {"crbm_slab_stats_data", &out->slab_stats_data}, {"crbm_slab_stats_model", &out->slab_stats_model}, {"crbm_slab_fe", &out->slab_fe}, {"crbm_gibbs", &out->gibbs},
      {"crbm_gibbs_sparse", &out->gibbs_sparse}, {"crbm_gibbs_sparse_stats", &out->gibbs_sparse_stats}, {"crbm_train_local", &out->train_local},
      {"crbm_stats_mfma_data", &out->stats_mfma_data},
      {"crbm_stats_mfma_model", &out->stats_mfma_model}, {"crbm_free_energy", &out->free_energy},
      {"crbm_hit_summary", &out->hit_summary}, {"crbm_motif_sites", &out->motif_sites},
      {"crbm_mutagenesis", &out->mutagenesis}, {"crbm_ais", &out->ais}, {"crbm_scan_sites", &out->scan_sites},
      {"crbm_scan_hist", &out->scan_hist}, {"crbm_variant_effects", &out->variant_effects}};
  for (auto& s : syms) {
    e = hipModuleGetFunction(s.f, out->module, s.name);
    if (e != hipSuccess) {
      *err = std::string("hipModuleGetFunction(") + s.name + "): " + hipGetErrorString(e);
      return -1;
    }
  }
  return 0;
}

template <typename Args>
inline hipError_t jit_launch(hipFunction_t f, const Args& args, unsigned gx, unsigned gy, unsigned block, unsigned lds,
                             hipStream_t stream) {
  Args copy = args;
  void* params[] = {&copy};
  if (lds > 48 * 1024) {
    static std::mutex mu;
    static std::unordered_map<hipFunction_t, unsigned> opted;
    std::lock_guard<std::mutex> lock(mu);
    unsigned& have = opted[f];
    if (lds > have) {
      (void)hipFuncSetAttribute(reinterpret_cast<const void*>(f), hipFuncAttributeMaxDynamicSharedMemorySize, (int)lds);
      (void)hipGetLastError();
      have = lds;
    }
  }
  return hipModuleLaunchKernel(f, gx, gy, 1, block, 1, 1, lds, stream, params, nullptr);
}

}
```

### crbm_amd/csrc/crbm_kernels.h

```cpp
#pragma once
#include <hip/hip_runtime.h>
#include <stdint.h>
#include "crbm_layout.h"

namespace crbm {

template <int I>
struct IC {
  static constexpr int value = I;
};

struct Philox4 {
  uint32_t v[4];
};

struct HalfFrag {
  uint32_t r[4];
};
#if defined(__clang__)
typedef float floatx4 __attribute__((ext_vector_type(4)));
__device__ __forceinline__ uint32_t xor3(uint32_t a, uint32_t b, uint32_t c) { return __builtin_amdgcn_bitop3_b32(a, b, c, 0x96); }
__device__ __forceinline__ uint32_t bitrev32(uint32_t x) { return __builtin_bitreverse32(x); }
__device__ __forceinline__ void store4_streaming(uint32_t* dst, uint32_t x, uint32_t y, uint32_t z, uint32_t w) {
  typedef uint32_t u4v __attribute__((ext_vector_type(4)));
// ... 970 lines not shown
      float* col = Pt + lane;
      if constexpr (C::POOL > 1) {
        if (valid) {
          const uint32_t* lrow = a.letters + (size_t)chain * a.LW;
          constexpr int NV = 4 * R::NQW;
          float p[NV], cb[NV], S[NV];
#pragma unroll
          for (int strand = 0; strand <= C::DS; ++strand) {
            auto zfun = [&](int pos, float (&z)[NV]) {
              const LetterWin<M> w = letter_window<M>(lrow, pos);
              conv_gather_quads<C, R::NQW>(Tf, strand ? revcomp_window<M>(w) : w, 4 * nt0, z);
            };
            pooled_probs<C::POOL, NV>(zfun, s, p, cb, S);
#pragma unroll
            for (int kl = 0; kl < KW; ++kl)
              if (16 * nt0 + kl < K) {
                const float ps = 16384.0f * p[kl];
                col[(size_t)(strand * KW + kl) * STATS_RS] = ps;
                if (SP && strand == 0) col[(size_t)((1 + C::DS) * KW + kl) * STATS_RS] = ps * (1.0f - S[kl]);
              }
          }
        } else {
#pragma unroll
          for (int r = 0; r < R::PARKED * KW; ++r) col[(size_t)r * STATS_RS] = 0.f;
        }
      } else
      if (valid) {
        const LetterWin<M> wl = letter_window<M>(gw + NPW * slot, e);
        float z[4 * R::NQW];
        conv_gather_quads<C, R::NQW>(Tf, wl, 4 * nt0, z);
#pragma unroll
        for (int kl = 0; kl < KW; ++kl)
          if (16 * nt0 + kl < K) {
            const float ps = fast_rcp(fmaf(exp_neg_x(z[kl]), STATS_PSCALE_INV, STATS_PSCALE_INV));
            col[(size_t)kl * STATS_RS] = ps;
            if (SP && !R::QDERIVE) col[(size_t)((1 + C::DS) * KW + kl) * STATS_RS] = fmaf(-ps * STATS_PSCALE_INV, ps, ps);
          }
        if (C::DS) {
          conv_gather_quads<C, R::NQW>(Tf, revcomp_window<M>(wl), 4 * nt0, z);
#pragma unroll
          for (int kl = 0; kl < KW; ++kl)
            if (16 * nt0 + kl < K)
              col[(size_t)(KW + kl) * STATS_RS] = fast_rcp(fmaf(exp_neg_x(z[kl]), STATS_PSCALE_INV, STATS_PSCALE_INV));
        }
      } else {
#pragma unroll
        for (int r = 0; r < R::PARKED * KW; ++r) col[(size_t)r * STATS_RS] = 0.f;
      }
    }
    __builtin_amdgcn_wave_barrier();
#pragma unroll
    for (int slot = 0; slot < 2; ++slot)
      if (G0 + slot < ngroups && !(a.debug & 1))
        stats_mfma_group<C, R, BYTE_LUT>(Pt, win + 2 * NPW * slot, lut, nt0, slot, acc);
    __builtin_amdgcn_wave_barrier();
  }
  if (a.debug & 8) return;
  stats_mfma_finish<C, SP>(sg, smem, nt0, bid, acc, vcount);
}

struct GibbsArgs {
  const float* tables;
  const float* tables_tf = nullptr;
  int32_t off_ws = 0;
  uint32_t* hm;
  uint32_t* hmp;
  uint32_t* vout;
  int32_t nchains, Lf, Lv, S;
  int32_t nvb, nhb;
  int32_t Lrow;
  int32_t LWs;
  FastDiv divVB, divHB, divRow, divLfw;
  int32_t steps;
  RngView rng;
  uint32_t* ones;
  unsigned long long* clock = nullptr;
  unsigned long long* timeline = nullptr;
  int32_t debug;
  int32_t nblocks;
  int32_t stats_off;
  StatsGeom sg;
};

__device__ __forceinline__ uint32_t sample_letter(float y0, float y1, float y2, float y3, float u) {
  const float mx = fmaxf(fmaxf(y0, y1), fmaxf(y2, y3));
  const float e0 = __builtin_amdgcn_exp2f(y0 - mx), e1 = __builtin_amdgcn_exp2f(y1 - mx), e2 = __builtin_amdgcn_exp2f(y2 - mx),
              e3 = __builtin_amdgcn_exp2f(y3 - mx);
  const float t = u * ((e0 + e1) + (e2 + e3));
  return (uint32_t)(t >= e0) + (uint32_t)(t >= e0 + e1) + (uint32_t)(t >= (e0 + e1) + e2);
}

template <class C>
__device__ __forceinline__ void topdown_bits(unsigned long long w, const char* tab, int q_base, float (&y)[4][4], int unit_base = 0) {
  constexpr int K = C::K;
  const char* tab_q = tab + ((size_t)q_base * K + unit_base) * 16;
  const char* idle = tab - K * 16;
  auto rows_of = [&](unsigned long long bits) { return bits ? tab_q + (__ffsll(bits) - 1) * 16 : idle; };
  auto fetch = [&](const char* p, float4 (&t)[4]) {
#pragma unroll
    for (int i = 0; i < 4; ++i) t[i] = *reinterpret_cast<const float4*>(p + (4 - i) * K * 16);
  };
  float4 cur[4];
  fetch(rows_of(w), cur);
  while (w) {
    w &= w - 1ull;
    float4 nxt[4];
    fetch(rows_of(w), nxt);
#pragma unroll
    for (int i = 0; i < 4; ++i) {
      y[i][0] += cur[i].x; y[i][1] += cur[i].y; y[i][2] += cur[i].z; y[i][3] += cur[i].w;
      cur[i] = nxt[i];
    }
  }
}

template <class C, bool SPARSE, bool STATS = false>
__device__ void gibbs_body(const GibbsArgs& a, int bid = -1) {
  constexpr int KP = C::KP, M = C::M, NW = C::NW, NCH = C::NCH;
  static_assert(SPARSE || C::DENSE, "no dense top-down tables for this model");
  using SR = StatsRole<C, false>;
  static_assert(!STATS || SR::NR == 1, "the fused statistics need all motifs of a position in one wave");
  constexpr int LTAB = SPARSE ? C::SP_TABLES : C::TABLES;
  HIP_DYNAMIC_SHARED(float, smem);
  const float* Tf = smem;
  const float* cv = smem + (SPARSE ? C::SP_C : C::OFF_C);
  uint32_t* hm = reinterpret_cast<uint32_t*>(smem + LTAB);
  uint32_t* hmp = hm + (size_t)a.S * a.Lrow * NW;
  uint32_t* let = hmp + (C::DS ? (size_t)a.S * a.Lrow * NW : 0);
  uint32_t* fixq = let + (size_t)a.S * a.LWs;
#ifdef CRBM_INLINE_EXACT_PATH
  constexpr bool DEFER = false;
#else
  constexpr bool DEFER = C::POOL == 1 && C::DS;
#endif

  bool tables_done = (a.debug & 1) != 0;
  auto copy_all_tables = [&]() {
    if (SPARSE) {
      copy_tables<C::TAB>(smem, a.tables_tf ? a.tables_tf : a.tables);
      copy_tables<C::WS * (1 + C::DS) + 4>(smem + C::SP_WS, a.tables + (a.tables_tf ? a.off_ws : C::OFF_WS));
    } else {
      copy_tables<C::TABLES>(smem, a.tables);
    }
    tables_done = true;
  };

  const int rowW = a.Lrow * NW;
  const uint32_t per = (uint32_t)(a.Lf * NW);
  const int ntiles = (a.nchains + a.S - 1) / a.S;
  if (bid < 0) bid = (int)blockIdx.x;
  if (a.clock && bid == 0 && threadIdx.x == 0) {
    a.clock[2] = realtime_ticks();
    a.clock[3] = shader_cycles();
  }
  if (a.timeline && bid == 0 && threadIdx.x == 0) a.timeline[0] = realtime_ticks();
  const int nblk = a.nblocks > 0 ? a.nblocks : (int)gridDim.x;
  int nset = 0;
  const int lane = threadIdx.x & 63, wave = threadIdx.x >> 6, nwaves = blockDim.x >> 6;
  float* sreg = nullptr;
  uint32_t* swin = nullptr;
  float* sPt = nullptr;
  floatx4 sacc[STATS ? SR::NACC : 1];
  float vcount = 0.f;
  if constexpr (STATS) {
    sreg = smem + a.stats_off;
    float* sslice = sreg + a.sg.off_slices + (size_t)wave * a.sg.slice;
    swin = reinterpret_cast<uint32_t*>(sslice + a.sg.off_win);
    sPt = sslice + a.sg.off_pt;
#pragma unroll
    for (int t = 0; t < SR::NACC; ++t) sacc[t] = floatx4{0.f, 0.f, 0.f, 0.f};
    stats_build_lut<false>(reinterpret_cast<uint32_t*>(sreg));
    for (int i = lane; i < SR::ROWS * STATS_RS; i += 64) sPt[i] = 0.f;
  }
  if (threadIdx.x == 0) fixq[0] = 0u;
  {
    const int padw = rowW - (int)per, front = (M - 1) * NW;
    for (int idx = threadIdx.x; idx < a.S * padw; idx += blockDim.x) {
      const int nl = idx / padw, e = idx - nl * padw;
      const int d = nl * rowW + (e < front ? e : e + (int)per);
      hm[d] = 0u;
      if (C::DS) hmp[d] = 0u;
    }
  }
  for (int tile = bid; tile < ntiles; tile += nblk) {
    const int n0 = tile * a.S;
    const int ns = min(a.S, a.nchains - n0);
    __syncthreads();
    if (!(a.debug & 2)) {
      const uint32_t nwords = (uint32_t)ns * per;
      auto lds_index = [&](uint32_t i) {
        const uint32_t nl = fastdiv_tile(i, a.divLfw);
        return nl * (uint32_t)rowW + (uint32_t)((M - 1) * NW) + (i - nl * per);
      };
      const size_t g0 = (size_t)n0 * per;
      if (((g0 | nwords) & 3u) == 0u) {
        constexpr int UN = 2;
        const uint4* src = reinterpret_cast<const uint4*>(a.hm + g0);
        const uint4* srcp = C::DS ? reinterpret_cast<const uint4*>(a.hmp + g0) : nullptr;
        for (uint32_t base0 = 0; base0 < nwords / 4; base0 += UN * blockDim.x) {
          const uint32_t base = base0 + threadIdx.x;
          uint4 t[UN], tp[UN];
#pragma unroll
          for (int u = 0; u < UN; ++u) {
            const uint32_t i4 = base + u * blockDim.x;
            if (i4 < nwords / 4) {
              t[u] = src[i4];
              if (C::DS) tp[u] = srcp[i4];
            }
          }
          if (!tables_done) copy_all_tables();
#pragma unroll
          for (int u = 0; u < UN; ++u) {
            const uint32_t i4 = base + u * blockDim.x;
            if (i4 < nwords / 4) {
              const uint32_t e[4] = {t[u].x, t[u].y, t[u].z, t[u].w};
              const uint32_t ep[4] = {tp[u].x, tp[u].y, tp[u].z, tp[u].w};
#pragma unroll
              for (int c = 0; c < 4; ++c) {
                const uint32_t d = lds_index(4 * i4 + c);
                hm[d] = e[c];
                if (C::DS) hmp[d] = ep[c];
              }
            }
          }
        }
      } else {
        constexpr int UN = 8;
        for (uint32_t base0 = 0; base0 < nwords; base0 += UN * blockDim.x) {
          const uint32_t base = base0 + threadIdx.x;
          uint32_t t[UN], tp[UN];
#pragma unroll
          for (int u = 0; u < UN; ++u) {
            const uint32_t i = base + u * blockDim.x;
            if (i < nwords) {
              t[u] = a.hm[g0 + i];
              if (C::DS) tp[u] = a.hmp[g0 + i];
            }
          }
          if (!tables_done) copy_all_tables();
#pragma unroll
          for (int u = 0; u < UN; ++u) {
            const uint32_t i = base + u * blockDim.x;
            if (i < nwords) {
              const uint32_t d = lds_index(i);
              hm[d] = t[u];
              if (C::DS) hmp[d] = tp[u];
            }
          }
        }
      }
    }
    if (!tables_done) copy_all_tables();
    for (int idx = threadIdx.x; idx < ns * a.LWs; idx += blockDim.x) let[idx] = 0u;
    auto resolve = [&](uint32_t e, int st, bool last) -> uint32_t {
      const uint32_t it = e & 0xFFFFFu, k = (e >> 20) & 0x7FFu, strand = e >> 31;
      const uint32_t nl = fastdiv_tile(it, a.divHB);
      const int s = (int)(it - nl * (uint32_t)a.nhb);
      const uint32_t gn = a.rng.seq_offset + (uint32_t)(n0 + nl);
      LetterWin<M> win = letter_window<M>(let + nl * (uint32_t)a.LWs, s);
      if (strand) win = revcomp_window<M>(win);
      const float* T = Tf + k;
      float z = 0.f;
#pragma unroll
      for (int g = 0; g < C::NG; ++g) {
        const uint32_t r = window_bits<C::M>(win, 2 * C::G * g) & (uint32_t)(C::ROWS - 1);
        const float t = T[((size_t)g * C::ROWS + r) * KP];
        z = g == 0 ? t : z + t;
      }
      const uint32_t g10 = k / 10u, i10 = k - 10u * g10, step = a.rng.step + (uint32_t)st;
      const Philox4 rc = philox4x32(gn, (uint32_t)s, rng_word2(KIND_CHAIN_H, strand, 0, g10), step, a.rng.seed_lo, a.rng.seed_hi);
      const Philox4 rf = philox4x32(gn, (uint32_t)s, rng_word2(KIND_CHAIN_H, strand, 1, g10), step, a.rng.seed_lo, a.rng.seed_hi);
      const float t = 4096.0f * fast_rcp(1.0f + exp_neg_x(z));
      const float frac = t - (float)philox_field12_dyn(rc, (int)i10);
      const uint32_t one = frac * 4096.0f > (float)philox_field12_dyn(rf, (int)i10) ? 1u : 0u;
      if (one) {
        const uint32_t bit = 1u << (k & 31u), w = k >> 5;
        if (last) { if (!(a.debug & 4)) atomicOr((strand ? a.hmp : a.hm) + (size_t)n0 * per + it * (uint32_t)NW + w, bit); }
        else atomicOr((strand ? hmp : hm) + (nl * (uint32_t)(rowW - (int)per) + it * (uint32_t)NW + (uint32_t)((M - 1) * NW)) + w, bit);
      }
      return one;
    };
    auto defer_units = [&](const uint32_t (&pending)[C::NGRP], uint32_t it, uint32_t strand, int st, bool last) -> uint32_t {
      uint32_t any = 0u, ones = 0u;
#pragma unroll
      for (int g = 0; g < C::NGRP; ++g) any |= pending[g];
      if (__any(any != 0u)) {
#pragma unroll
        for (int g = 0; g < C::NGRP; ++g) {
          uint32_t m = pending[g];
          while (m) {
            const uint32_t i = (uint32_t)__ffs(m) - 1u;
            m &= m - 1u;
            const uint32_t e = it | ((10u * (uint32_t)g + i) << 20) | (strand << 31);
            const uint32_t slot = atomicAdd(&fixq[0], 1u);
            if (slot < (uint32_t)FIXQ_CAP) fixq[2 + slot] = e;
            else ones += resolve(e, st, last);
          }
        }
      }
      return ones;
    };
    auto drain_queue = [&](int st, bool last) {
      if (last) wait_vector_memory();
      __syncthreads();
      const uint32_t nq = min(fixq[0], (uint32_t)FIXQ_CAP);
      for (uint32_t e = threadIdx.x; e < nq; e += blockDim.x) {
        const uint32_t one = resolve(fixq[2 + e], st, last);
        if (last) nset += (int)one;
      }
    };
    for (int st = 0; st < a.steps; ++st) {
      __syncthreads();
      if (threadIdx.x == 0) fixq[0] = 0u;
      for (uint32_t it = threadIdx.x; it < (uint32_t)(ns * a.nvb); it += blockDim.x) {
        const uint32_t nl = fastdiv_tile(it, a.divVB);
        const int pb = (int)(it - nl * (uint32_t)a.nvb);
        const int p0 = 4 * pb;
        float y[4][4];
#pragma unroll
        for (int i = 0; i < 4; ++i) { y[i][0] = cv[0]; y[i][1] = cv[1]; y[i][2] = cv[2]; y[i][3] = cv[3]; }
        if constexpr (!SPARSE) {
          constexpr int NMV = (M + 3 + 3) / 4;
#pragma unroll
          for (int strand = 0; strand <= C::DS; ++strand) {
            const uint4* mrow = reinterpret_cast<const uint4*>((strand ? hmp : hm) + (size_t)nl * a.Lrow + p0);
            const char* Tv = reinterpret_cast<const char*>(smem + (strand ? C::OFF_TVR : C::OFF_TV));
            uint32_t off[4 * NMV][NCH];
#pragma unroll
            for (int v4 = 0; v4 < NMV; ++v4) {
              const uint4 mm = mrow[v4];
              const uint32_t m4[4] = {mm.x, mm.y, mm.z, mm.w};
#pragma unroll
              for (int e = 0; e < 4; ++e)
#pragma unroll
                for (int ch = 0; ch < NCH; ++ch)
                  off[4 * v4 + e][ch] = (5 * ch >= 4 ? (m4[e] >> (5 * ch - 4)) : (m4[e] << (4 - 5 * ch))) & 0x1F0u;
            }
#pragma unroll
            for (int jr = 0; jr < M; ++jr)
#pragma unroll
              for (int ch = 0; ch < NCH; ++ch)
#pragma unroll
                for (int i = 0; i < 4; ++i) {
                  const float4 t = *reinterpret_cast<const float4*>(Tv + (jr * NCH + ch) * 512 + off[i + jr][ch]);
                  y[i][0] += t.x; y[i][1] += t.y; y[i][2] += t.z; y[i][3] += t.w;
                }
          }
        } else {
          constexpr int NSLOT = M + 3;
          constexpr int PPW = NW == 1 ? 64 / C::K : 1;
          constexpr int NWORD = (NSLOT + PPW - 1) / PPW;
#pragma unroll
          for (int strand = 0; strand <= C::DS; ++strand) {
            const uint32_t* mrow = (strand ? hmp : hm) + ((size_t)nl * a.Lrow + p0) * NW;
            const char* tab = reinterpret_cast<const char*>(smem + (strand ? C::SP_WSR : C::SP_WS));
            if constexpr (NW == 1) {
              constexpr int NMV = (NSLOT + 3) / 4;
              uint32_t m[4 * NMV];
#pragma unroll
              for (int v4 = 0; v4 < NMV; ++v4) {
                const uint4 mm = reinterpret_cast<const uint4*>(mrow)[v4];
                m[4 * v4] = mm.x; m[4 * v4 + 1] = mm.y; m[4 * v4 + 2] = mm.z; m[4 * v4 + 3] = mm.w;
              }
#pragma unroll
              for (int wi = 0; wi < NWORD; ++wi) {
                unsigned long long w = 0ull;
#pragma unroll
                for (int t = 0; t < PPW; ++t)
                  if (wi * PPW + t < NSLOT) w |= (unsigned long long)m[wi * PPW + t] << (t * C::K);
                topdown_bits<C>(w, tab, wi * PPW, y);
              }
            } else {
#pragma unroll 1
              for (int q = 0; q < NSLOT; ++q) {
                if constexpr (NW == 2) {
                  const uint2 mm = *reinterpret_cast<const uint2*>(mrow + 2 * q);
                  topdown_bits<C>((unsigned long long)mm.x | ((unsigned long long)mm.y << 32), tab, q, y);
                } else {
#pragma unroll
                  for (int w2 = 0; 2 * w2 < NW; ++w2) {
                    const uint32_t lo = mrow[NW * q + 2 * w2], hi = 2 * w2 + 1 < NW ? mrow[NW * q + 2 * w2 + 1] : 0u;
                    topdown_bits<C>((unsigned long long)lo | ((unsigned long long)hi << 32), tab, q, y, 64 * w2);
                  }
                }
              }
            }
          }
        }
        const Philox4 r = philox4x32(a.rng.seq_offset + (uint32_t)(n0 + nl), (uint32_t)pb,
                                        rng_word2(KIND_CHAIN_V, 0, 0, 0), a.rng.step + (uint32_t)st,
                                        a.rng.seed_lo, a.rng.seed_hi);
        uint32_t byte = 0u;
#pragma unroll
        for (int i = 0; i < 4; ++i) {
          const uint32_t l = sample_letter(y[i][0], y[i][1], y[i][2], y[i][3], u01(r.v[i]));
          byte |= (p0 + i < a.Lv ? l : 0u) << (2 * i);
        }
        reinterpret_cast<unsigned char*>(let + (size_t)nl * a.LWs)[pb] = (unsigned char)byte;
      }
      __syncthreads();
      bool fused_pass = false;
      if constexpr (STATS) if (st == a.steps - 1) {
        fused_pass = true;
        constexpr int KW = SR::KW;
        const int GPC = a.sg.GPC, ngl = ns * GPC;
        for (int u = wave; 2 * u < ngl; u += nwaves) {
          const int G0 = 2 * u;
          constexpr int NPW = C::NPW;
          if (lane < 8 * NPW) {
            const int G = G0 + lane / (4 * NPW), w = (lane >> 2) % NPW;
            int gi = 0;
            uint32_t word = 0u;
            if (G < ngl) {
              const uint32_t nl = fastdiv_tile((uint32_t)G, a.sg.divGPC);
              gi = G - (int)nl * GPC;
              if (2 * gi + w < a.LWs) word = let[(size_t)nl * a.LWs + 2 * gi + w];
            }
            vcount += stats_window_piece<NPW>(reinterpret_cast<unsigned short*>(swin), lane, word, G < ngl, gi, GPC, a.Lv);
          }
          __builtin_amdgcn_wave_barrier();
          {
            const int slot = lane >> 5, G = G0 + slot;
            bool valid = G < ngl;
            uint32_t nl = 0u;
            int s = 0;
            if (valid) {
              nl = fastdiv_tile((uint32_t)G, a.sg.divGPC);
              s = 32 * (G - (int)nl * GPC) + (lane & 31);
              valid = s < a.Lf;
            }
            float* col = sPt + lane;
            if (valid) {
              const uint32_t gn = a.rng.seq_offset + (uint32_t)(n0 + nl);
              const LetterWin<M> win = letter_window<M>(let + (size_t)nl * a.LWs, s);
#pragma unroll
              for (int strand = 0; strand <= C::DS; ++strand) {
                float x[KP], p[KP];
                conv_gather<C>(Tf, strand ? revcomp_window<M>(win) : win, x);
                uint32_t mask[NW];
                uint32_t pend[C::NGRP];
                sample_hidden<C, 2, DEFER>(x, gn, (uint32_t)s, KIND_CHAIN_H, (uint32_t)strand, a.rng,
                                           a.rng.step + (uint32_t)st, mask, p, pend);
                uint32_t* dst = (strand ? a.hmp : a.hm) + (size_t)(n0 + nl) * per + (size_t)s * NW;
#pragma unroll
                for (int w = 0; w < NW; ++w) {
                  if (!(a.debug & 4)) store1_streaming(dst + w, mask[w]);
                  nset += __popc(mask[w]);
                }
                if constexpr (DEFER) nset += (int)defer_units(pend, nl * (uint32_t)a.nhb + (uint32_t)s, (uint32_t)strand, st, true);
#pragma unroll
                for (int k = 0; k < C::K; ++k) col[(size_t)(strand * KW + k) * STATS_RS] = p[k];
              }
            } else {
#pragma unroll
              for (int r = 0; r < SR::KINDS * KW; ++r) col[(size_t)r * STATS_RS] = 0.f;
            }
          }
          __builtin_amdgcn_wave_barrier();
#pragma unroll
          for (int slot = 0; slot < 2; ++slot)
            if (G0 + slot < ngl)
              stats_mfma_group<C, SR, false>(sPt, swin + 2 * C::NPW * slot, reinterpret_cast<const uint32_t*>(sreg), 0, slot, sacc);
          __builtin_amdgcn_wave_barrier();
        }
      }
      if (!fused_pass) {
      for (uint32_t it = threadIdx.x; it < (uint32_t)(ns * a.nhb); it += blockDim.x) {
        const uint32_t nl = fastdiv_tile(it, a.divHB);
        const int s = (int)(it - nl * (uint32_t)a.nhb);
        const uint32_t gn = a.rng.seq_offset + (uint32_t)(n0 + nl);
        const uint32_t* lrow = let + nl * (uint32_t)a.LWs;
        const LetterWin<M> win = letter_window<M>(lrow, s);
#pragma unroll
        for (int strand = 0; strand <= C::DS; ++strand) {
          float x[KP], p[KP];
          uint32_t mask[NW], pend[C::NGRP];
          if constexpr (C::POOL > 1) {
            auto zfun = [&](int pos, float (&z)[KP]) {
              const LetterWin<M> w = letter_window<M>(lrow, pos);
              conv_gather<C>(Tf, strand ? revcomp_window<M>(w) : w, z);
            };
            float cb[KP], S[KP], u[KP];
            pooled_probs<C::POOL, KP>(zfun, s, p, cb, S);
            hidden_uniforms24<C>(gn, (uint32_t)(s - s % C::POOL), KIND_CHAIN_H, (uint32_t)strand, a.rng, a.rng.step + (uint32_t)st, u);
            pooled_sample<C>(p, cb, u, mask);
          } else {
          conv_gather<C>(Tf, strand ? revcomp_window<M>(win) : win, x);
          sample_hidden<C, 0, DEFER>(x, gn, (uint32_t)s, KIND_CHAIN_H, (uint32_t)strand, a.rng,
                                     a.rng.step + (uint32_t)st, mask, p, pend);
          }
          if (st == a.steps - 1) {
            uint32_t* dst = (strand ? a.hmp : a.hm) + (size_t)n0 * per + it * (uint32_t)NW;
#pragma unroll
            for (int w = 0; w < NW; ++w) {
              if (!(a.debug & 4)) store1_streaming(dst + w, mask[w]);
              nset += __popc(mask[w]);
            }
          } else {
            uint32_t* dst = (strand ? hmp : hm) + (nl * (uint32_t)(rowW - (int)per) + it * (uint32_t)NW + (uint32_t)((M - 1) * NW));
#pragma unroll
            for (int w = 0; w < NW; ++w) dst[w] = mask[w];
          }
          if constexpr (DEFER) {
            const uint32_t ones = defer_units(pend, it, (uint32_t)strand, st, st == a.steps - 1);
            if (st == a.steps - 1) nset += (int)ones;
          }
        }
      }
      }
      if constexpr (DEFER) drain_queue(st, st == a.steps - 1);
    }
    if (a.steps == 0) __syncthreads();
    if (a.steps == 0 && !(a.debug & 4)) {
      const uint32_t nwords = (uint32_t)ns * per;
      const size_t g0 = (size_t)n0 * per;
      auto lds_index = [&](uint32_t i) {
        const uint32_t nl = fastdiv_tile(i, a.divLfw);
        return nl * (uint32_t)rowW + (uint32_t)((M - 1) * NW) + (i - nl * per);
      };
      if (((g0 | nwords) & 3u) == 0u) {
        for (uint32_t i4 = threadIdx.x; i4 < nwords / 4; i4 += blockDim.x) {
          const uint32_t d0 = lds_index(4 * i4), d1 = lds_index(4 * i4 + 1), d2 = lds_index(4 * i4 + 2), d3 = lds_index(4 * i4 + 3);
          store4_streaming(a.hm + g0 + 4 * (size_t)i4, hm[d0], hm[d1], hm[d2], hm[d3]);
          if (C::DS) store4_streaming(a.hmp + g0 + 4 * (size_t)i4, hmp[d0], hmp[d1], hmp[d2], hmp[d3]);
        }
      } else {
        for (uint32_t i = threadIdx.x; i < nwords; i += blockDim.x) {
          const uint32_t d = lds_index(i);
          a.hm[g0 + i] = hm[d];
          if (C::DS) a.hmp[g0 + i] = hmp[d];
        }
      }
    }
    if (a.vout && !(a.debug & 4))
      for (int idx = threadIdx.x; idx < ns * a.LWs; idx += blockDim.x)
        a.vout[(size_t)n0 * a.LWs + idx] = let[idx];
  }
  if (a.ones) {
    const float tot = wave_sum((float)nset);
    if ((threadIdx.x & 63) == 0) a.ones[bid * (blockDim.x >> 6) + (threadIdx.x >> 6)] = (uint32_t)tot;
  }
  if (a.clock && bid == 0 && threadIdx.x == 0) {
    a.clock[0] += realtime_ticks() - a.clock[2];
    a.clock[1] += shader_cycles() - a.clock[3];
  }
  if (a.timeline && bid == 0 && threadIdx.x == 0) a.timeline[1] = realtime_ticks();
  if constexpr (STATS) stats_mfma_finish<C, false>(a.sg, smem, 0, bid, sacc, vcount);
}

struct TrainLocalArgs {
  GibbsArgs g;
  StatsMfmaArgs d;
};

template <class C>
__device__ void train_local_body(const TrainLocalArgs& a) {
  if constexpr (C::FUSE_STATS) {
    const int nG = a.g.nblocks, nD = a.d.nblocks, m = min(nG, nD), b = (int)blockIdx.x;
    const bool chain = b < 2 * m ? !(b & 1) : nG > nD;
    const int idx = b < 2 * m ? b >> 1 : b - m;
    if (chain) gibbs_body<C, true, true>(a.g, idx);
    else stats_mfma_body<C, true, false>(a.d, idx);
  }
}

struct FeArgs {
  const float* tables;
  const uint32_t* letters;
  int32_t n, L, Lh, LW;
  float* fe;
  float* fem;
};

__device__ __forceinline__ float softplus_of_z(float z) {
  const float t = __builtin_amdgcn_exp2f(-fabsf(z));
  const float series = t * (1.0f - t * (0.5f - t * (0.33333334f - 0.25f * t)));
  const float vialog = 0.6931471805599453f * __builtin_amdgcn_logf(1.0f + t);
  return fmaxf(x_of_z(z), 0.f) + (t < 0.03125f ? series : vialog);
}

template <class C>
__device__ void free_energy_body(const FeArgs& a) {
  constexpr int KP = C::KP, K = C::K, M = C::M;
  HIP_DYNAMIC_SHARED(float, smem);
  float* Tf = smem;
  copy_tables<C::TAB>(Tf, a.tables + C::OFF_TF);
  __syncthreads();
  const int lane = threadIdx.x & 63, wave = threadIdx.x >> 6, nwaves = blockDim.x >> 6;
  const float* cg = a.tables + C::OFF_C;
  const float c0 = LN2 * cg[0], c1 = LN2 * cg[1], c2 = LN2 * cg[2], c3 = LN2 * cg[3];
  for (int nn = blockIdx.x * nwaves + wave; nn < a.n; nn += gridDim.x * nwaves) {
    const uint32_t* row = a.letters + (size_t)nn * a.LW;
    float acc[KP];
#pragma unroll
    for (int q = 0; q < KP; ++q) acc[q] = 0.f;
    if constexpr (C::POOL > 1) {
      for (int g0 = lane * C::POOL; g0 < a.Lh; g0 += 64 * C::POOL)
#pragma unroll
        for (int strand = 0; strand <= C::DS; ++strand) {
          auto zfun = [&](int pos, float (&z)[KP]) {
            const LetterWin<M> w = letter_window<M>(row, pos);
            conv_gather<C>(Tf, strand ? revcomp_window<M>(w) : w, z);
          };
          pooled_softplus<C::POOL, KP>(zfun, g0, acc, K);
        }
    } else
    for (int s = lane; s < a.Lh; s += 64) {
      const LetterWin<M> win = letter_window<M>(row, s);
      float x[KP];
      conv_gather<C>(Tf, win, x);
#pragma unroll
      for (int q = 0; q < K; ++q) acc[q] += softplus_of_z(x[q]);
      if (C::DS) {
        conv_gather<C>(Tf, revcomp_window<M>(win), x);
#pragma unroll
        for (int q = 0; q < K; ++q) acc[q] += softplus_of_z(x[q]);
      }
    }
    float cs = 0.f;
    for (int p = lane; p < a.L; p += 64) {
      const uint32_t l = (row[p >> 4] >> (2 * (p & 15))) & 3u;
      cs += l == 0u ? c0 : l == 1u ? c1 : l == 2u ? c2 : c3;
    }
    cs = wave_sum(cs);
    float tot = 0.f;
#pragma unroll
    for (int q = 0; q < K; ++q) {
      const float v = wave_sum(acc[q]);
      tot += v;
      if (lane == 0 && a.fem) a.fem[(size_t)nn * K + q] = -v - cs;
    }
    if (lane == 0 && a.fe) a.fe[nn] = (-tot - cs) / (float)a.L;
  }
}

constexpr float HIT_FX = 1073741824.0f;
struct HitArgs {
  const float* tables;
  const uint32_t* letters;
  int32_t n, L, Lh, LW;
  float* hmax;
  float* hsum;
  unsigned long long* hsum_fx;
  float inv_Lh;
// ... 1632 lines not shown
```

### crbm_amd/csrc/crbm_plan.h

```cpp
#pragma once

#include "crbm_layout.h"

#include <algorithm>
#include <cmath>
#include <cstdlib>

namespace crbm {

inline int env_int(const char* name, int dflt) {
  const char* v = getenv(name);
  return (v && *v) ? atoi(v) : dflt;
}

inline int solo_group(int K, int M, int ds, int G, int pool) {
  const int forced = env_int("CRBM_GROUP_SOLO", 0);
  if (forced >= 1 && forced <= 4) return forced;
  if (!model_shape(K, M, ds, G, pool).FUSE_STATS) return G;
  return std::max(G, choose_group(K, M, ds, 48 * 1024));
}

struct GibbsGeom {
  int S, threads, grid, lds;
};
// ... 25 lines not shown
      const double score = util * balance * (0.4 + 0.6 * occupancy) - 1e-4 * S;
      if (score > best_score) {
        best_score = score;
        best = GibbsGeom{S, threads, (int)std::min(ntiles, (double)num_cu * blocks_cu), gl.lds_bytes};
        if (threads <= 256) best_occupancy = occupancy;
      }
    }
  }
  const int forceG = env_int("CRBM_GIBBS_GRID", 0);
  if (forceG > 0) best.grid = forceG;
  return best;
}

struct PartPlan {
  int parts, part_chains;
  GibbsGeom geom;
};
inline PartPlan plan_chain_parts(const ModelShape& ms, int Lf, int B, int num_cu) {
  PartPlan one{1, B, GibbsGeom{0, 0, 0, 0}};
  const int forced = env_int("CRBM_CHAIN_PARTS", 0);
  if (forced == 1 || B < 2) return one;
  const int parts = forced >= 2 ? std::min(forced, 4) : 2;
  const int half = (B + parts - 1) / parts;
  GibbsGeom g = choose_gibbs_geometry(ms, Lf, half, num_cu, true, false);
  if (g.lds <= 0) return one;
  const int tiles = (B + g.S - 1) / g.S, tiles_part = (tiles + parts - 1) / parts;
  const int blocks_cu = std::max(1, std::min((160 * 1024) / g.lds, 1024 / g.threads));
  if (forced < 2) {
    const double items = (double)B * Lf * ms.K * (1 + ms.DS);
    if (blocks_cu < 2 || tiles_part < num_cu || items > 256e6) return one;
  }
  if (tiles_part < 1) return one;
  PartPlan p{parts, tiles_part * g.S, g};
  p.geom.grid = std::min(tiles_part, num_cu * blocks_cu);
  return p;
}

inline bool model_needs_big(const ModelShape& ms, int Lf, int B, int num_cu) {
  if (env_int("CRBM_FORCE_BIG", 0)) return true;
  if (ms.K > MAX_MOTIFS || ms.M > MAX_MOTIF_LENGTH) return true;
  if (choose_gibbs_geometry(ms, Lf, B, num_cu, true).lds <= 0) return true;
  for (int want_sp = 0; want_sp <= 1; ++want_sp) {
    const int tabs = ms.TAB * 4;
    const StatsMfmaLayout st = stats_mfma_layout(ms, want_sp, Lf, 0, tabs, true);
    if (st.threads > 1024 || std::max(st.region_floats * 4 + tabs, st.combine_bytes) > 160 * 1024) return true;
  }
  return false;
}

inline int gibbs_block_bound(int threads) { return threads > 512 ? 1024 : threads > 256 ? 512 : 256; }

inline int gibbs_wpe_hint(const GibbsGeom& g) {
  if (g.lds <= 0) return 0;
  const int blocks_cu = std::max(1, std::min((160 * 1024) / g.lds, 2048 / g.threads));
  const int wpe = std::max(1, blocks_cu * (g.threads / 64) / 4);
  return wpe < 4 ? wpe : 0;
}

inline int slab_choose(int K, int M, int ds, int pool, int Lf, int* G_out, ModelShape* ms_out) {
  const int want = std::max(10, std::min(env_int("CRBM_SLAB_MOTIFS", 60), 64));
  const int first = K <= want ? K : want / 10 * 10;
  for (int cand : {first, 40, 30, 20, 10}) {
    if (cand > K || (cand != first && cand >= first)) continue;
    int G = env_int("CRBM_SLAB_GROUP", 0);
    if (G < 1 || G > 4) {
      const int budget = env_int("CRBM_SLAB_TABLE_BUDGET", 26 * 1024);
      G = choose_group(cand, M, ds, budget);
      if (G == 1) G = choose_group(cand, M, ds, std::max(budget, 48 * 1024));
    }
    const ModelShape ms = model_shape(cand, M, ds, G, pool);
    bool fit = true;
    for (int want_sp = 0; want_sp <= 1 && fit; ++want_sp) {
      const int tabs = ms.TAB * 4;
      const StatsMfmaLayout st = stats_mfma_layout(ms, want_sp, Lf, 0, tabs, true);
      if (st.threads > 1024 || std::max(st.region_floats * 4 + tabs, st.combine_bytes) > 160 * 1024) fit = false;
    }
    if (fit) { *G_out = G; *ms_out = ms; return cand; }
  }
  return 0;
}

struct ChainGeom { GibbsLayout gl = {}; int threads = 0, grid = 0; bool on() const { return threads > 0; } };

struct LaunchPlan {
  bool big = false;
  int G = 0, GS = 0;
  ModelShape ms = {}, ms_solo = {};
  bool has_dense = false;
  ChainGeom chain[2];
  ChainGeom solo;
  ChainGeom part;
  int chain_parts = 1, part_chains = 0;
  int gibbs_wpe = 0, gibbs_tb = 256;
  int slab_K = 0, slab_G = 0;
  ModelShape slab_ms = {};
  const char* slab_note = nullptr;
  const char* refusal = nullptr;
};

inline const ChainGeom& plain_geom(const LaunchPlan& p, int variant, bool parts = true) {
  if (variant == 1 && parts && p.chain_parts > 1) return p.part;
  if (variant == 1 && p.solo.on()) return p.solo;
  return p.chain[variant];
}

inline LaunchPlan plan_launches(int K, int M, int ds, int A, int pool, int Lf, int B, int num_cu) {
  LaunchPlan p;
  p.G = env_int("CRBM_GROUP", 0);
  if (p.G < 1 || p.G > 4) p.G = choose_group(K, M, ds, env_int("CRBM_TABLE_BUDGET", 26 * 1024));
  p.ms = model_shape(K, M, ds, p.G, pool);
  p.GS = p.G; p.ms_solo = p.ms;
  p.part_chains = B;
  p.big = (K > MAX_MOTIFS || M > MAX_MOTIF_LENGTH || A != 4) ? true : model_needs_big(p.ms, Lf, B, num_cu);
  if (p.big) {
    if (env_int("CRBM_SLAB_STATS", 1) == 0) p.slab_note = "CRBM_SLAB_STATS=0";
    else if (A != 4 || M > MAX_MOTIF_LENGTH) p.slab_note = "other alphabet, or motifs beyond 64 letters";
    else {
      p.slab_K = slab_choose(K, M, ds, pool, Lf, &p.slab_G, &p.slab_ms);
      if (!p.slab_K) p.slab_note = "no slab of this motif length fits the LDS";
    }
    return p;
  }
  p.has_dense = p.ms.DENSE != 0;
  for (int v = p.has_dense ? 0 : 1; v < 2; ++v) {
    const GibbsGeom geom = choose_gibbs_geometry(p.ms, Lf, B, num_cu, v == 1);
    if (geom.lds <= 0) { p.refusal = "model too large for the LDS-resident Gibbs kernel"; continue; }
    p.chain[v] = ChainGeom{gibbs_layout(p.ms, Lf, geom.S, v == 1), geom.threads, geom.grid};
    if (v == 1) p.gibbs_wpe = gibbs_wpe_hint(geom);
  }
  const PartPlan parts = plan_chain_parts(p.ms, Lf, B, num_cu);
  p.chain_parts = parts.parts;
  if (parts.parts > 1) {
    p.part_chains = parts.part_chains;
    p.part = ChainGeom{gibbs_layout(p.ms, Lf, parts.geom.S, true), parts.geom.threads, parts.geom.grid};
  }
  p.GS = parts.parts > 1 ? p.G : solo_group(K, M, ds, p.G, pool);
  p.ms_solo = model_shape(K, M, ds, p.GS, pool);
  GibbsGeom solo = choose_gibbs_geometry(p.ms_solo, Lf, B, num_cu, true, true);
  if (solo.lds <= 0 && p.GS != p.G) {
    p.GS = p.G; p.ms_solo = p.ms;
    solo = choose_gibbs_geometry(p.ms_solo, Lf, B, num_cu, true, true);
  }
  if (solo.lds > 0 && (p.GS != p.G || solo.threads != p.chain[1].threads || solo.S != p.chain[1].gl.S || solo.grid != p.chain[1].grid))
    p.solo = ChainGeom{gibbs_layout(p.ms_solo, Lf, solo.S, true), solo.threads, solo.grid};
  int threads = 0;
  for (const ChainGeom* g : {&p.chain[0], &p.chain[1], &p.solo, &p.part}) threads = std::max(threads, g->threads);
  p.gibbs_tb = gibbs_block_bound(threads);
  return p;
}

}
```

### include/crbm_amd.h

```cpp
#ifndef CRBM_AMD_H
#define CRBM_AMD_H

#include <stdint.h>

#ifdef __cplusplus
extern "C" {
#endif

#define CRBM_AMD_ABI_VERSION 5

typedef enum crbm_status {
  CRBM_OK = 0,
  CRBM_ERR_INVALID = -1,
  CRBM_ERR_HIP = -2,
  CRBM_ERR_NOT_ONEHOT = -3,
  CRBM_ERR_NOT_BINARY = -4,
  CRBM_ERR_RCCL = -5,
  CRBM_ERR_NO_GPU = -6,
  CRBM_ERR_IPC_TIMEOUT = -7
} crbm_status;

typedef struct crbm_config {
  int32_t num_motifs;
  int32_t motif_length;
// ... 48 lines not shown
int crbm_time_train(crbm_handle* h, int32_t start, int32_t end, int32_t launches, float* total_ms);

int crbm_h_given_v(crbm_handle* h, const float* v, int32_t n, int32_t L, int32_t flip,
                   uint32_t rng_step, float* act, float* prob, float* sample);
int crbm_v_given_h(crbm_handle* h, const float* hid, const float* hid_prime, int32_t n,
                   int32_t Lh, uint32_t rng_step, float* act, float* prob, float* sample);

int crbm_hit_probs(crbm_handle* h, const float* v, int32_t n, int32_t L, float* out);
int crbm_free_energy(crbm_handle* h, const float* v, int32_t n, int32_t L, float* out);
int crbm_free_energy_per_motif(crbm_handle* h, const float* v, int32_t n, int32_t L, float* out);
int crbm_eval_data(crbm_handle* h, const float* v, int32_t n, int32_t L, float* mfe, float* nmh);
int crbm_eval_params(crbm_handle* h, float* twn, float* ic, float* medic);

int crbm_hit_probs_codes(crbm_handle* h, const uint8_t* codes, int32_t n, int32_t L, float* out);
int crbm_hit_probs_resident(crbm_handle* h, int32_t start, int32_t end, float* out);
int crbm_free_energy_codes(crbm_handle* h, const uint8_t* codes, int32_t n, int32_t L, float* fe, float* fe_per_motif);
int crbm_free_energy_resident(crbm_handle* h, int32_t start, int32_t end, float* fe, float* fe_per_motif);
int crbm_eval_data_resident(crbm_handle* h, int32_t start, int32_t end, float* mfe, float* nmh);
int crbm_eval_epoch_resident(crbm_handle* h, int32_t batchsize, double* mean_fe, double* mean_nmh);
int crbm_hit_summary(crbm_handle* h, const float* v, int32_t n, int32_t L, float* hit_max, float* hit_mean,
                     float* position_mean);
int crbm_hit_summary_codes(crbm_handle* h, const uint8_t* codes, int32_t n, int32_t L, float* hit_max,
                           float* hit_mean, float* position_mean);
int crbm_hit_summary_resident(crbm_handle* h, int32_t start, int32_t end, float* hit_max, float* hit_mean,
                              float* position_mean);

typedef struct crbm_site {
  int32_t seq, motif, start, strand;
  float prob;
} crbm_site;
int crbm_motif_sites(crbm_handle* h, const float* v, int32_t n, int32_t L, float threshold, int64_t capacity,
                     crbm_site* sites, int64_t* count, int32_t* best_start, int32_t* best_strand, float* best_prob);
int crbm_motif_sites_codes(crbm_handle* h, const uint8_t* codes, int32_t n, int32_t L, float threshold, int64_t capacity,
                           crbm_site* sites, int64_t* count, int32_t* best_start, int32_t* best_strand, float* best_prob);
int crbm_motif_sites_resident(crbm_handle* h, int32_t start, int32_t end, float threshold, int64_t capacity,
                              crbm_site* sites, int64_t* count, int32_t* best_start, int32_t* best_strand,
                              float* best_prob);

int crbm_scan_sites_codes(crbm_handle* h, const uint8_t* codes, int64_t T, float threshold, int64_t capacity,
                          crbm_site* sites, int64_t* count);

int crbm_scan_histogram_codes(crbm_handle* h, const uint8_t* codes, int64_t T, float lo, float hi, int32_t nbins,
                              uint64_t* counts, int64_t* windows);

int crbm_variant_effects_codes(crbm_handle* h, const uint8_t* codes, int64_t T, int64_t nvar, const int64_t* pos,
                               const uint8_t* alt, float* dfe, float* dfe_per_motif, int32_t* windows);

int crbm_mutagenesis(crbm_handle* h, const float* v, int32_t n, int32_t L, float* dfe, float* pll);
int crbm_mutagenesis_codes(crbm_handle* h, const uint8_t* codes, int32_t n, int32_t L, float* dfe, float* pll);
int crbm_mutagenesis_resident(crbm_handle* h, int32_t start, int32_t end, float* dfe, float* pll);

int crbm_ais(crbm_handle* h, int32_t L, int32_t runs, uint32_t run_offset, const float* betas, int32_t nbetas,
             int32_t t0, int32_t t1, const float* base_c, uint64_t seed, uint8_t* state, float* logw);

#define CRBM_UNIQUE_ID_BYTES 128
int crbm_comm_unique_id(uint8_t id[CRBM_UNIQUE_ID_BYTES]);
int crbm_comm_init(crbm_handle* h, const uint8_t id[CRBM_UNIQUE_ID_BYTES], int32_t nranks, int32_t rank);
int crbm_comm_destroy(crbm_handle* h);
int crbm_comm_broadcast_state(crbm_handle* h, int32_t root);
#define CRBM_IPC_HANDLE_BYTES 64
int crbm_ipc_export(crbm_handle* h, uint8_t handle[CRBM_IPC_HANDLE_BYTES]);
int crbm_ipc_attach(crbm_handle* h, const uint8_t* handles, int32_t nranks, int32_t rank);
int crbm_ipc_detach(crbm_handle* h);
int crbm_ipc_status(crbm_handle* h, int32_t* timed_out);
int crbm_sums_count(const crbm_handle* h);
int crbm_train_local(crbm_handle* h, const float* D, int32_t n, int32_t L, float* sums_out);
int crbm_train_apply(crbm_handle* h, const float* sums_in, int32_t L_data);
int crbm_time_allreduce(crbm_handle* h, int32_t launches, float* total_ms);

typedef struct crbm_launch_info {
  int32_t nq;
  int32_t group;
  int32_t gibbs_grid, gibbs_block, gibbs_seqs_per_tile, gibbs_lds_bytes;
  int32_t stats_grid_x, stats_grid_y, stats_block, stats_lds_bytes;
  int32_t gibbs_sparse;
  int32_t activity_ppm;
  int32_t stats_fused;
  int32_t chain_parts;
  int32_t mutagenesis_route;
} crbm_launch_info;
int crbm_get_launch_info(const crbm_handle* h, crbm_launch_info* out);
int crbm_copy_bandwidth(crbm_handle* h, int64_t bytes, int32_t reps, float* gb_per_s);
int crbm_last_shader_clock(crbm_handle* h, float* mhz);
int64_t crbm_gibbs_state_bytes(const crbm_handle* h);

#ifdef __cplusplus
}
#endif
#endif
```

Baseline: 58250 8192-chain batch Gibbs steps/s (summed over GPUs).

## JIT-specialise Gibbs kernels with compile-time launch geometry constants

```diff
diff --git a/__graft_entry__.py b/__graft_entry__.py
--- a/__graft_entry__.py
+++ b/__graft_entry__.py
@@ -30,13 +30,17 @@
     (33, 17, 0, 1, 33), (64, 32, 1, 1, 33), (20, 40, 1, 1, 33), (4, 64, 1, 1, 33), (100, 15, 0, 1, 33), (130, 7, 1, 1, 33),
     (256, 4, 0, 1, 33), (6, 7, 1, 2, 34), (10, 15, 0, 4, 36), (5, 8, 1, 3, 33), (300, 10, 0, 1, 33), (150, 6, 1, 2, 34),
     (10, 15, 0, 1, 64), (10, 15, 0, 1, 32), (20, 40, 1, 1, 64), (20, 40, 1, 1, 32)]]
+GEOMETRY_SHAPES = [dict(num_motifs=k, motif_length=m, doublestranded=ds, batchsize=b, fantasy_hidden_len=lf,
+                        env=dict(CRBM_GEOM="2", CRBM_GIBBS_S=str(s)))
+                   for (k, m, ds, lf, b, s) in [(10, 15, 0, 186, 8, 4), (10, 15, 0, 185, 8, 4), (10, 15, 0, 185, 6, 2), (10, 15, 1, 50, 6, 2), (40, 6, 0, 30, 4, 4),
+                                                (10, 15, 0, 186, 9, 4), (10, 15, 1, 50, 8, 2)]]
 
 
 def build():
     from crbm_amd.csrc import build as hip_build
     hip_build.build(verbose=True)
     hip_build.prune_cache()
-    hip_build.precompile(PRECOMPILE + STATISTICS_SHAPES, verbose=False)
+    hip_build.precompile(PRECOMPILE + STATISTICS_SHAPES + GEOMETRY_SHAPES, verbose=False)
     from oracle import build_cpu
     build_cpu.build(verbose=True)
     import crbm_amd
diff --git a/crbm_amd/_lib.py b/crbm_amd/_lib.py
--- a/crbm_amd/_lib.py
+++ b/crbm_amd/_lib.py
@@ -131,6 +131,7 @@
     "crbm_get_launch_info": (_I32, [_H, ctypes.POINTER(CrbmLaunchInfo)]),
     "crbm_copy_bandwidth": (_I32, [_H, ctypes.c_int64, _I32, _F]),
     "crbm_last_shader_clock": (_I32, [_H, _F]),
+    "crbm_geometry_launches": (_I32, [_H, _I64P, _I64P]),
     "crbm_gibbs_state_bytes": (ctypes.c_int64, [_H]),
 }
 
diff --git a/crbm_amd/csrc/build.py b/crbm_amd/csrc/build.py
--- a/crbm_amd/csrc/build.py
+++ b/crbm_amd/csrc/build.py
@@ -79,7 +79,17 @@
                               doublestranded=int(c.get("doublestranded", 0)), batchsize=c.get("batchsize", 20),
                               cd_k=1, pooling=c.get("pooling", 1), fantasy_hidden_len=c.get("fantasy_hidden_len", 200),
                               learning_rate=0.1, momentum=0.9, rho=0.01, lambda_rate=0.1, seed=0, device=0, reserved=0)
-        rc = lib.crbm_precompile(ctypes.byref(cfg))
+        knobs = c.get("env", {})
+        saved = {k: os.environ.get(k) for k in knobs}
+        os.environ.update(knobs)
+        try:
+            rc = lib.crbm_precompile(ctypes.byref(cfg))
+        finally:
+            for k, v in saved.items():
+                if v is None:
+                    os.environ.pop(k, None)
+                else:
+                    os.environ[k] = v
         if rc != 0:
             raise RuntimeError("precompile failed for %s: %s" % (c, lib.crbm_last_error(None).decode()))
         if verbose:
diff --git a/crbm_amd/csrc/crbm_api.hip b/crbm_amd/csrc/crbm_api.hip
--- a/crbm_amd/csrc/crbm_api.hip
+++ b/crbm_amd/csrc/crbm_api.hip
@@ -197,6 +197,8 @@
   unsigned long long* d_probe = nullptr;
   unsigned long long probe_base[2] = {0, 0}, probe_last[2] = {0, 0};
   bool probe_on = false;
+  JitGeoKernels jg;
+  long long geo_launches[2] = {0, 0};
   unsigned long long* d_timeline = nullptr;
   int timeline_cap = 0, timeline_next = 0;
   unsigned long long ipc_timeout_ticks = 0;
@@ -441,6 +443,19 @@
 }
 
 StatsGeom stats_geom(const StatsMfmaLayout& st, float* partials, long ngroups, int lds_bytes);
+
+JitGeo jit_geo(const GeoSpec& s, int Lf) {
+  JitGeo j;
+  if (!s.on()) return j;
+  j.S = s.gl.S; j.Lf = Lf; j.Lv = s.gl.Lv; j.Lrow = s.gl.Lrow; j.LWs = s.gl.LWs; j.nvb = s.gl.nvb; j.nhb = s.gl.nhb;
+  j.threads = s.threads; j.nchains = s.nchains; j.grid = s.grid; j.aligned = s.aligned ? 1 : 0; j.group = s.group;
+  return j;
+}
+
+hipFunction_t geo_kernel(const GeoSpec& spec, hipFunction_t fn, const ChainGeom& g, const GibbsArgs& a) {
+  if (!fn || a.steps < 1 || a.debug || a.timeline) return nullptr;
+  return spec.serves(g.gl, g.threads, a.nblocks, a.nchains) && a.Lf == spec.gl.nhb ? fn : nullptr;
+}
 
 int prepare_gibbs(crbm_handle* h, const ChainGeom& g, int steps, ReduceArgs* model_reduce, GibbsArgs* out, unsigned* lds_out) {
   const GibbsLayout& gl = g.gl;
@@ -580,18 +595,21 @@
     if (p > 0) ap.clock = nullptr;
     if (h->d_timeline && h->timeline_next < h->timeline_cap) ap.timeline = h->d_timeline + 2 * (size_t)(h->timeline_next++);
     ap.nblocks = (int)grid;
+    hipFunction_t fn = geo_kernel(plan.geo_plain, h->jg.gibbs_sparse, plan.part, ap);
+    h->geo_launches[fn ? 1 : 0] += 1;
+    if (!fn) fn = h->jk.gibbs_sparse;
     if (p > 0) {
       PartWorker* w = h->part_worker[p];
       {
         std::lock_guard<std::mutex> lock(w->mu);
-        w->jobs.push_back(PartJob{h->jk.gibbs_sparse, ap, grid, threads, lds, (unsigned long long)(stagger_ticks * p)});
+        w->jobs.push_back(PartJob{fn, ap, grid, threads, lds, (unsigned long long)(stagger_ticks * p)});
       }
       w->cv.notify_one();
       continue;
     }
     const bool calibrate = first_of_fork && !h->cal_pending;
     if (calibrate) HIPCHK(hipEventRecord(h->ev_cal0, h->part_stream[0]));
-    HIPCHK(jit_launch(h->jk.gibbs_sparse, ap, grid, 1, threads, lds, h->part_stream[0]));
+    HIPCHK(jit_launch(fn, ap, grid, 1, threads, lds, h->part_stream[0]));
     if (calibrate) {
       HIPCHK(hipEventRecord(h->ev_cal1, h->part_stream[0]));
       h->cal_pending = true;
@@ -620,6 +638,12 @@
   h->nset_slots = g.grid * (g.threads / 64);
   if (plain && h->d_timeline && h->timeline_next < h->timeline_cap) a.timeline = h->d_timeline + 2 * (size_t)(h->timeline_next++);
   hipFunction_t fn = model_reduce ? h->jk.gibbs_sparse_stats : (h->variant ? h->jk.gibbs_sparse : h->jk.gibbs);
+  if (h->variant == 1) {
+    hipFunction_t geo = model_reduce ? geo_kernel(h->plan.geo_fused, h->jg.gibbs_sparse_stats, g, a)
+                                     : geo_kernel(h->plan.geo_plain, h->jg.gibbs_sparse, g, a);
+    if (geo) fn = geo;
+    h->geo_launches[geo ? 1 : 0] += 1;
+  }
   HIPCHK(jit_launch(fn, a, (unsigned)g.grid, 1, (unsigned)g.threads, lds, s));
   h->gibbs_step += (uint32_t)steps;
   h->launches_since_read += 1;
@@ -966,7 +990,9 @@
     t.g.sg.lds_floats = (int)(lds / 4);
     t.d.sg.lds_floats = (int)(lds / 4);
     h->nset_slots = g.grid * (g.threads / 64);
-    HIPCHK(jit_launch(h->jk.train_local, t, (unsigned)(g.grid + d.grid), 1, (unsigned)g.threads, lds, h->stream));
+    hipFunction_t fn = h->variant == 1 ? geo_kernel(h->plan.geo_fused, h->jg.train_local, g, t.g) : nullptr;
+    h->geo_launches[fn ? 1 : 0] += 1;
+    HIPCHK(jit_launch(fn ? fn : h->jk.train_local, t, (unsigned)(g.grid + d.grid), 1, (unsigned)g.threads, lds, h->stream));
     h->gibbs_step += (uint32_t)h->cfg.cd_k;
     h->launches_since_read += 1;
     return launch_reduce_pair(h, pair, publish);
@@ -1379,6 +1405,10 @@
     rc_jit = jit_compile(p.ms.K, p.ms.M, p.ms.DS, p.G, p.GS, p.ms.POOL, p.gibbs_wpe, p.gibbs_tb, &code, &cached, &file, &err);
   else if (p.slab_K > 0)
     rc_jit = jit_compile(p.slab_K, p.ms.M, p.ms.DS, p.slab_G, p.slab_G, p.slab_ms.POOL, 0, 256, &code, &cached, &file, &err, true);
+  if (rc_jit == 0 && !p.big && (p.geo_plain.on() || p.geo_fused.on())) {
+    const int Lf = cfg->fantasy_hidden_len > 0 ? cfg->fantasy_hidden_len : 200;
+    rc_jit = jit_compile_geo(p.ms.K, p.ms.M, p.ms.DS, p.ms.POOL, p.gibbs_wpe, jit_geo(p.geo_plain, Lf), jit_geo(p.geo_fused, Lf), &code, &cached, &file, &err);
+  }
   if (rc_jit != 0) {
     g_create_error = err;
     return CRBM_ERR_HIP;
@@ -1438,6 +1468,11 @@
     std::string err;
     if (jit_load(hh->K, hh->M, hh->ds, plan.G, plan.GS, hh->ms().POOL, plan.gibbs_wpe, plan.gibbs_tb, &hh->jk, &err) != 0) {
       g_create_error = "kernel specialisation failed: " + err;
+      return bail(CRBM_ERR_HIP);
+    }
+    if (hh->variant == 1 &&
+        jit_load_geo(hh->K, hh->M, hh->ds, hh->ms().POOL, plan.gibbs_wpe, jit_geo(plan.geo_plain, hh->Lf), jit_geo(plan.geo_fused, hh->Lf), &hh->jg, &err) != 0) {
+      g_create_error = "kernel specialisation (launch geometry) failed: " + err;
       return bail(CRBM_ERR_HIP);
     }
   }
@@ -1556,6 +1591,7 @@
   }
   h->ais_betas.release(); h->ais_base.release(); h->ais_logw.release(); h->ais_state.release(); h->hist.release();
   if (h->jk.module) (void)hipModuleUnload(h->jk.module);
+  if (h->jg.module) (void)hipModuleUnload(h->jg.module);
   if (h->ev0) (void)hipEventDestroy(h->ev0);
   if (h->ev1) (void)hipEventDestroy(h->ev1);
   if (h->ev_fork) (void)hipEventDestroy(h->ev_fork);
@@ -3134,6 +3170,13 @@
   return CRBM_OK;
 }
 
+int crbm_geometry_launches(const crbm_handle* h, int64_t* compiled_in, int64_t* run_time) {
+  if (!h) return CRBM_ERR_INVALID;
+  if (compiled_in) *compiled_in = h->geo_launches[1];
+  if (run_time) *run_time = h->geo_launches[0];
+  return CRBM_OK;
+}
+
 int crbm_last_shader_clock(crbm_handle* h, float* mhz) {
   ENTER();
   ARGCHK(mhz, "null argument");
diff --git a/crbm_amd/csrc/crbm_jit.h b/crbm_amd/csrc/crbm_jit.h
--- a/crbm_amd/csrc/crbm_jit.h
+++ b/crbm_amd/csrc/crbm_jit.h
@@ -101,15 +101,58 @@
   return buf;
 }
 
+struct JitGeo {
+  int S = 0, Lf = 0, Lv = 0, Lrow = 0, LWs = 0, nvb = 0, nhb = 0, threads = 0, nchains = 0, grid = 0, aligned = 0, group = 0;
+  bool on() const { return threads > 0; }
+};
+
+inline std::string jit_geo_stub(int K, int M, int DS, int POOL, int gibbs_wpe, const JitGeo& plain, const JitGeo& fused) {
+  char attr[96];
+  if (gibbs_wpe > 0) snprintf(attr, sizeof(attr), "__attribute__((amdgpu_waves_per_eu(1, %d)))", gibbs_wpe);
+  else snprintf(attr, sizeof(attr), "__attribute__((amdgpu_waves_per_eu(4)))");
+  std::string s = "#define CRBM_SLAB_KERNELS 0\n#include \"crbm_kernels.h\"\n#ifndef CRBM_GIBBS_ATTR\n#define CRBM_GIBBS_ATTR ";
+  s += attr;
+  s += "\n#endif\n";
+  char buf[1024];
+  auto policy = [&](const char* name, const char* cfg, const JitGeo& g) {
+    snprintf(buf, sizeof(buf), "using %s = crbm::Cfg<%d, %d, %d, %d, %d>;\nusing %sGeo = crbm::GeomCT<%d, %d, %d, %d, %d, %d, %d, %d, %d, %d, %s>;\n",
+             cfg, K, M, DS, g.group, POOL, name, g.S, g.Lf, g.Lv, g.Lrow, g.LWs, g.nvb, g.nhb, g.threads, g.nchains, g.grid, g.aligned ? "true" : "false");
+    s += buf;
+  };
+  if (plain.on()) {
+    policy("Plain", "PlainCfg", plain);
+    snprintf(buf, sizeof(buf), "extern \"C\" __global__ void __launch_bounds__(%d) CRBM_GIBBS_ATTR crbm_gibbs_sparse_geo(crbm::GibbsArgs a) { crbm::gibbs_geo_body<PlainCfg, PlainGeo>(a); }\n", plain.threads);
+    s += buf;
+  }
+  if (fused.on()) {
+    policy("Fused", "FusedCfg", fused);
+    snprintf(buf, sizeof(buf),
+             "extern \"C\" __global__ void __launch_bounds__(%d) CRBM_GIBBS_ATTR crbm_gibbs_sparse_stats_geo(crbm::GibbsArgs a) { if constexpr (FusedCfg::FUSE_STATS) crbm::gibbs_body<FusedCfg, true, true, FusedGeo>(a); }\n"
+             "extern \"C\" __global__ void __launch_bounds__(%d) CRBM_GIBBS_ATTR crbm_train_local_geo(crbm::TrainLocalArgs a) { crbm::train_local_body<FusedCfg, FusedGeo>(a); }\n",
+             fused.threads, fused.threads);
+    s += buf;
+  }
+  return s;
+}
+
+inline int jit_compile_source(const std::string& stub, std::vector<char>* code, bool* from_cache, std::string* cache_file, std::string* err);
+
 inline int jit_compile(int K, int M, int DS, int G, int GS, int POOL, int gibbs_wpe, int gibbs_tb, std::vector<char>* code, bool* from_cache,
                        std::string* cache_file, std::string* err, bool slab = false) {
+  return jit_compile_source(jit_stub(K, M, DS, G, GS, POOL, gibbs_wpe, gibbs_tb, slab), code, from_cache, cache_file, err);
+}
+inline int jit_compile_geo(int K, int M, int DS, int POOL, int gibbs_wpe, const JitGeo& plain, const JitGeo& fused, std::vector<char>* code,
+                           bool* from_cache, std::string* cache_file, std::string* err) {
+  return jit_compile_source(jit_geo_stub(K, M, DS, POOL, gibbs_wpe, plain, fused), code, from_cache, cache_file, err);
+}
+
+inline int jit_compile_source(const std::string& stub, std::vector<char>* code, bool* from_cache, std::string* cache_file, std::string* err) {
   const std::string dir = jit_source_dir();
   std::string kernels, layout;
   if (!jit_read_file(dir + "/crbm_kernels.h", &kernels) || !jit_read_file(dir + "/crbm_layout.h", &layout)) {
     *err = "kernel sources not found in " + dir + " (set CRBM_KERNEL_SRC_DIR)";
     return -1;
   }
-  const std::string stub = jit_stub(K, M, DS, G, GS, POOL, gibbs_wpe, gibbs_tb, slab);
   std::vector<std::string> opts = {"--offload-arch=gfx950", "-O3", "-std=c++17", "-ffp-contract=off",
                                    "-I" + dir, "-I/opt/rocm/include"};
   if (const char* e = getenv("CRBM_JIT_DEFINES")) {
@@ -199,6 +242,34 @@
   return 0;
 }
 
+struct JitGeoKernels {
+  hipModule_t module = nullptr;
+  hipFunction_t gibbs_sparse = nullptr, gibbs_sparse_stats = nullptr, train_local = nullptr;
+};
+inline int jit_load_geo(int K, int M, int DS, int POOL, int gibbs_wpe, const JitGeo& plain, const JitGeo& fused, JitGeoKernels* out, std::string* err) {
+  if (!plain.on() && !fused.on()) return 0;
+  std::vector<char> code;
+  bool cached = false;
+  if (jit_compile_geo(K, M, DS, POOL, gibbs_wpe, plain, fused, &code, &cached, nullptr, err) != 0) return -1;
+  hipError_t e = hipModuleLoadData(&out->module, code.data());
+  if (e != hipSuccess) {
+    *err = std::string("hipModuleLoadData: ") + hipGetErrorString(e);
+    return -1;
+  }
+  struct { bool want; const char* name; hipFunction_t* f; } syms[] = {
+      {plain.on(), "crbm_gibbs_sparse_geo", &out->gibbs_sparse}, {fused.on(), "crbm_gibbs_sparse_stats_geo", &out->gibbs_sparse_stats},
+      {fused.on(), "crbm_train_local_geo", &out->train_local}};
+  for (auto& s : syms) {
+    if (!s.want) continue;
+    e = hipModuleGetFunction(s.f, out->module, s.name);
+    if (e != hipSuccess) {
+      *err = std::string("hipModuleGetFunction(") + s.name + "): " + hipGetErrorString(e);
+      return -1;
+    }
+  }
+  return 0;
+}
+
 template <typename Args>
 inline hipError_t jit_launch(hipFunction_t f, const Args& args, unsigned gx, unsigned gy, unsigned block, unsigned lds,
                              hipStream_t stream) {
diff --git a/crbm_amd/csrc/crbm_kernels.h b/crbm_amd/csrc/crbm_kernels.h
--- a/crbm_amd/csrc/crbm_kernels.h
+++ b/crbm_amd/csrc/crbm_kernels.h
@@ -1076,6 +1076,44 @@
   StatsGeom sg;
 };
 
+struct GeomRT {
+  static constexpr bool CT = false, PROF = true, ALIGNED = false, ONE = false;
+  const GibbsArgs& a;
+  __device__ __forceinline__ explicit GeomRT(const GibbsArgs& a_) : a(a_) {}
+  __device__ __forceinline__ int S() const { return a.S; }
+  __device__ __forceinline__ int Lf() const { return a.Lf; }
+  __device__ __forceinline__ int Lv() const { return a.Lv; }
+  __device__ __forceinline__ int Lrow() const { return a.Lrow; }
+  __device__ __forceinline__ int LWs() const { return a.LWs; }
+  __device__ __forceinline__ int nvb() const { return a.nvb; }
+  __device__ __forceinline__ int nhb() const { return a.nhb; }
+  __device__ __forceinline__ int nchains() const { return a.nchains; }
+  __device__ __forceinline__ uint32_t threads() const { return blockDim.x; }
+  __device__ __forceinline__ int nblk() const { return a.nblocks > 0 ? a.nblocks : (int)gridDim.x; }
+  __device__ __forceinline__ uint32_t div_vb(uint32_t i) const { return fastdiv_tile(i, a.divVB); }
+  __device__ __forceinline__ uint32_t div_hb(uint32_t i) const { return fastdiv_tile(i, a.divHB); }
+  template <int NW> __device__ __forceinline__ uint32_t div_lfw(uint32_t i) const { return fastdiv_tile(i, a.divLfw); }
+};
+template <int S_, int LF_, int LV_, int LROW_, int LWS_, int NVB_, int NHB_, int TB_, int NCHAINS_, int GRID_, bool ALIGNED_>
+struct GeomCT {
+  static_assert(S_ >= 1 && NCHAINS_ % S_ == 0 && GRID_ >= 1 && GRID_ <= NCHAINS_ / S_ && TB_ % 64 == 0, "GeomCT: full tiles only");
+  static constexpr bool CT = true, PROF = false, ALIGNED = ALIGNED_, ONE = GRID_ == NCHAINS_ / S_;
+  __device__ __forceinline__ explicit GeomCT(const GibbsArgs&) {}
+  __device__ __forceinline__ constexpr int S() const { return S_; }
+  __device__ __forceinline__ constexpr int Lf() const { return LF_; }
+  __device__ __forceinline__ constexpr int Lv() const { return LV_; }
+  __device__ __forceinline__ constexpr int Lrow() const { return LROW_; }
+  __device__ __forceinline__ constexpr int LWs() const { return LWS_; }
+  __device__ __forceinline__ constexpr int nvb() const { return NVB_; }
+  __device__ __forceinline__ constexpr int nhb() const { return NHB_; }
+  __device__ __forceinline__ constexpr int nchains() const { return NCHAINS_; }
+  __device__ __forceinline__ constexpr uint32_t threads() const { return TB_; }
+  __device__ __forceinline__ constexpr int nblk() const { return GRID_; }
+  __device__ __forceinline__ uint32_t div_vb(uint32_t i) const { return i / (uint32_t)NVB_; }
+  __device__ __forceinline__ uint32_t div_hb(uint32_t i) const { return i / (uint32_t)NHB_; }
+  template <int NW> __device__ __forceinline__ uint32_t div_lfw(uint32_t i) const { return i / (uint32_t)(LF_ * NW); }
+};
+
 __device__ __forceinline__ uint32_t sample_letter(float y0, float y1, float y2, float y3, float u) {
   const float mx = fmaxf(fmaxf(y0, y1), fmaxf(y2, y3));
   const float e0 = __builtin_amdgcn_exp2f(y0 - mx), e1 = __builtin_amdgcn_exp2f(y1 - mx), e2 = __builtin_amdgcn_exp2f(y2 - mx),
@@ -1108,8 +1146,11 @@
   }
 }
 
-template <class C, bool SPARSE, bool STATS = false>
+template <class C, bool SPARSE, bool STATS = false, class GP = GeomRT>
 __device__ void gibbs_body(const GibbsArgs& a, int bid = -1) {
+  const GP g(a);
+  const int dbg = GP::PROF ? a.debug : 0;
+  const uint32_t TB = g.threads();
   constexpr int KP = C::KP, M = C::M, NW = C::NW, NCH = C::NCH;
   static_assert(SPARSE || C::DENSE, "no dense top-down tables for this model");
   using SR = StatsRole<C, false>;
@@ -1119,16 +1160,16 @@
   const float* Tf = smem;
   const float* cv = smem + (SPARSE ? C::SP_C : C::OFF_C);
   uint32_t* hm = reinterpret_cast<uint32_t*>(smem + LTAB);
-  uint32_t* hmp = hm + (size_t)a.S * a.Lrow * NW;
-  uint32_t* let = hmp + (C::DS ? (size_t)a.S * a.Lrow * NW : 0);
-  uint32_t* fixq = let + (size_t)a.S * a.LWs;
+  uint32_t* hmp = hm + (size_t)g.S() * g.Lrow() * NW;
+  uint32_t* let = hmp + (C::DS ? (size_t)g.S() * g.Lrow() * NW : 0);
+  uint32_t* fixq = let + (size_t)g.S() * g.LWs();
 #ifdef CRBM_INLINE_EXACT_PATH
   constexpr bool DEFER = false;
 #else
   constexpr bool DEFER = C::POOL == 1 && C::DS;
 #endif
 
-  bool tables_done = (a.debug & 1) != 0;
+  bool tables_done = (dbg & 1) != 0;
   auto copy_all_tables = [&]() {
     if (SPARSE) {
       copy_tables<C::TAB>(smem, a.tables_tf ? a.tables_tf : a.tables);
@@ -1139,18 +1180,20 @@
     tables_done = true;
   };
 
-  const int rowW = a.Lrow * NW;
-  const uint32_t per = (uint32_t)(a.Lf * NW);
-  const int ntiles = (a.nchains + a.S - 1) / a.S;
+  const int rowW = g.Lrow() * NW;
+  const uint32_t per = (uint32_t)(g.Lf() * NW);
+  const int ntiles = (g.nchains() + g.S() - 1) / g.S();
   if (bid < 0) bid = (int)blockIdx.x;
-  if (a.clock && bid == 0 && threadIdx.x == 0) {
-    a.clock[2] = realtime_ticks();
-    a.clock[3] = shader_cycles();
-  }
-  if (a.timeline && bid == 0 && threadIdx.x == 0) a.timeline[0] = realtime_ticks();
-  const int nblk = a.nblocks > 0 ? a.nblocks : (int)gridDim.x;
+  if constexpr (GP::PROF) {
+    if (a.clock && bid == 0 && threadIdx.x == 0) {
+      a.clock[2] = realtime_ticks();
+      a.clock[3] = shader_cycles();
+    }
+    if (a.timeline && bid == 0 && threadIdx.x == 0) a.timeline[0] = realtime_ticks();
+  }
+  const int nblk = g.nblk();
   int nset = 0;
-  const int lane = threadIdx.x & 63, wave = threadIdx.x >> 6, nwaves = blockDim.x >> 6;
+  const int lane = threadIdx.x & 63, wave = threadIdx.x >> 6, nwaves = TB >> 6;
   float* sreg = nullptr;
   uint32_t* swin = nullptr;
   float* sPt = nullptr;
@@ -1169,34 +1212,34 @@
   if (threadIdx.x == 0) fixq[0] = 0u;
   {
     const int padw = rowW - (int)per, front = (M - 1) * NW;
-    for (int idx = threadIdx.x; idx < a.S * padw; idx += blockDim.x) {
+    for (int idx = threadIdx.x; idx < g.S() * padw; idx += TB) {
       const int nl = idx / padw, e = idx - nl * padw;
       const int d = nl * rowW + (e < front ? e : e + (int)per);
       hm[d] = 0u;
       if (C::DS) hmp[d] = 0u;
     }
   }
-  for (int tile = bid; tile < ntiles; tile += nblk) {
-    const int n0 = tile * a.S;
-    const int ns = min(a.S, a.nchains - n0);
+  for (int tile = bid; GP::ONE ? tile == bid : tile < ntiles; tile += nblk) {
+    const int n0 = tile * g.S();
+    const int ns = GP::CT ? g.S() : min(g.S(), g.nchains() - n0);
     __syncthreads();
-    if (!(a.debug & 2)) {
+    if (!(dbg & 2)) {
       const uint32_t nwords = (uint32_t)ns * per;
       auto lds_index = [&](uint32_t i) {
-        const uint32_t nl = fastdiv_tile(i, a.divLfw);
+        const uint32_t nl = g.template div_lfw<NW>(i);
         return nl * (uint32_t)rowW + (uint32_t)((M - 1) * NW) + (i - nl * per);
       };
       const size_t g0 = (size_t)n0 * per;
-      if (((g0 | nwords) & 3u) == 0u) {
+      if (GP::CT ? GP::ALIGNED : ((g0 | nwords) & 3u) == 0u) {
         constexpr int UN = 2;
         const uint4* src = reinterpret_cast<const uint4*>(a.hm + g0);
         const uint4* srcp = C::DS ? reinterpret_cast<const uint4*>(a.hmp + g0) : nullptr;
-        for (uint32_t base0 = 0; base0 < nwords / 4; base0 += UN * blockDim.x) {
+        for (uint32_t base0 = 0; base0 < nwords / 4; base0 += UN * TB) {
           const uint32_t base = base0 + threadIdx.x;
           uint4 t[UN], tp[UN];
 #pragma unroll
           for (int u = 0; u < UN; ++u) {
-            const uint32_t i4 = base + u * blockDim.x;
+            const uint32_t i4 = base + u * TB;
             if (i4 < nwords / 4) {
               t[u] = src[i4];
               if (C::DS) tp[u] = srcp[i4];
@@ -1205,7 +1248,7 @@
           if (!tables_done) copy_all_tables();
 #pragma unroll
           for (int u = 0; u < UN; ++u) {
-            const uint32_t i4 = base + u * blockDim.x;
+            const uint32_t i4 = base + u * TB;
             if (i4 < nwords / 4) {
               const uint32_t e[4] = {t[u].x, t[u].y, t[u].z, t[u].w};
               const uint32_t ep[4] = {tp[u].x, tp[u].y, tp[u].z, tp[u].w};
@@ -1220,12 +1263,12 @@
         }
       } else {
         constexpr int UN = 8;
-        for (uint32_t base0 = 0; base0 < nwords; base0 += UN * blockDim.x) {
+        for (uint32_t base0 = 0; base0 < nwords; base0 += UN * TB) {
           const uint32_t base = base0 + threadIdx.x;
           uint32_t t[UN], tp[UN];
 #pragma unroll
           for (int u = 0; u < UN; ++u) {
-            const uint32_t i = base + u * blockDim.x;
+            const uint32_t i = base + u * TB;
             if (i < nwords) {
               t[u] = a.hm[g0 + i];
               if (C::DS) tp[u] = a.hmp[g0 + i];
@@ -1234,7 +1277,7 @@
           if (!tables_done) copy_all_tables();
 #pragma unroll
           for (int u = 0; u < UN; ++u) {
-            const uint32_t i = base + u * blockDim.x;
+            const uint32_t i = base + u * TB;
             if (i < nwords) {
               const uint32_t d = lds_index(i);
               hm[d] = t[u];
@@ -1245,13 +1288,13 @@
       }
     }
     if (!tables_done) copy_all_tables();
-    for (int idx = threadIdx.x; idx < ns * a.LWs; idx += blockDim.x) let[idx] = 0u;
+    for (int idx = threadIdx.x; idx < ns * g.LWs(); idx += TB) let[idx] = 0u;
     auto resolve = [&](uint32_t e, int st, bool last) -> uint32_t {
       const uint32_t it = e & 0xFFFFFu, k = (e >> 20) & 0x7FFu, strand = e >> 31;
-      const uint32_t nl = fastdiv_tile(it, a.divHB);
-      const int s = (int)(it - nl * (uint32_t)a.nhb);
+      const uint32_t nl = g.div_hb(it);
+      const int s = (int)(it - nl * (uint32_t)g.nhb());
       const uint32_t gn = a.rng.seq_offset + (uint32_t)(n0 + nl);
-      LetterWin<M> win = letter_window<M>(let + nl * (uint32_t)a.LWs, s);
+      LetterWin<M> win = letter_window<M>(let + nl * (uint32_t)g.LWs(), s);
       if (strand) win = revcomp_window<M>(win);
       const float* T = Tf + k;
       float z = 0.f;
@@ -1269,7 +1312,7 @@
       const uint32_t one = frac * 4096.0f > (float)philox_field12_dyn(rf, (int)i10) ? 1u : 0u;
       if (one) {
         const uint32_t bit = 1u << (k & 31u), w = k >> 5;
-        if (last) { if (!(a.debug & 4)) atomicOr((strand ? a.hmp : a.hm) + (size_t)n0 * per + it * (uint32_t)NW + w, bit); }
+        if (last) { if (!(dbg & 4)) atomicOr((strand ? a.hmp : a.hm) + (size_t)n0 * per + it * (uint32_t)NW + w, bit); }
         else atomicOr((strand ? hmp : hm) + (nl * (uint32_t)(rowW - (int)per) + it * (uint32_t)NW + (uint32_t)((M - 1) * NW)) + w, bit);
       }
       return one;
@@ -1298,7 +1341,7 @@
       if (last) wait_vector_memory();
       __syncthreads();
       const uint32_t nq = min(fixq[0], (uint32_t)FIXQ_CAP);
-      for (uint32_t e = threadIdx.x; e < nq; e += blockDim.x) {
+      for (uint32_t e = threadIdx.x; e < nq; e += TB) {
         const uint32_t one = resolve(fixq[2 + e], st, last);
         if (last) nset += (int)one;
       }
@@ -1306,9 +1349,9 @@
     for (int st = 0; st < a.steps; ++st) {
       __syncthreads();
       if (threadIdx.x == 0) fixq[0] = 0u;
-      for (uint32_t it = threadIdx.x; it < (uint32_t)(ns * a.nvb); it += blockDim.x) {
-        const uint32_t nl = fastdiv_tile(it, a.divVB);
-        const int pb = (int)(it - nl * (uint32_t)a.nvb);
+      for (uint32_t it = threadIdx.x; it < (uint32_t)(ns * g.nvb()); it += TB) {
+        const uint32_t nl = g.div_vb(it);
+        const int pb = (int)(it - nl * (uint32_t)g.nvb());
         const int p0 = 4 * pb;
         float y[4][4];
 #pragma unroll
@@ -1317,7 +1360,7 @@
           constexpr int NMV = (M + 3 + 3) / 4;
 #pragma unroll
           for (int strand = 0; strand <= C::DS; ++strand) {
-            const uint4* mrow = reinterpret_cast<const uint4*>((strand ? hmp : hm) + (size_t)nl * a.Lrow + p0);
+            const uint4* mrow = reinterpret_cast<const uint4*>((strand ? hmp : hm) + (size_t)nl * g.Lrow() + p0);
             const char* Tv = reinterpret_cast<const char*>(smem + (strand ? C::OFF_TVR : C::OFF_TV));
             uint32_t off[4 * NMV][NCH];
 #pragma unroll
@@ -1346,7 +1389,7 @@
           constexpr int NWORD = (NSLOT + PPW - 1) / PPW;
 #pragma unroll
           for (int strand = 0; strand <= C::DS; ++strand) {
-            const uint32_t* mrow = (strand ? hmp : hm) + ((size_t)nl * a.Lrow + p0) * NW;
+            const uint32_t* mrow = (strand ? hmp : hm) + ((size_t)nl * g.Lrow() + p0) * NW;
             const char* tab = reinterpret_cast<const char*>(smem + (strand ? C::SP_WSR : C::SP_WS));
             if constexpr (NW == 1) {
               constexpr int NMV = (NSLOT + 3) / 4;
@@ -1388,9 +1431,9 @@
 #pragma unroll
         for (int i = 0; i < 4; ++i) {
           const uint32_t l = sample_letter(y[i][0], y[i][1], y[i][2], y[i][3], u01(r.v[i]));
-          byte |= (p0 + i < a.Lv ? l : 0u) << (2 * i);
-        }
-        reinterpret_cast<unsigned char*>(let + (size_t)nl * a.LWs)[pb] = (unsigned char)byte;
+          byte |= (p0 + i < g.Lv() ? l : 0u) << (2 * i);
+        }
+        reinterpret_cast<unsigned char*>(let + (size_t)nl * g.LWs())[pb] = (unsigned char)byte;
       }
       __syncthreads();
       bool fused_pass = false;
@@ -1408,9 +1451,9 @@
             if (G < ngl) {
               const uint32_t nl = fastdiv_tile((uint32_t)G, a.sg.divGPC);
               gi = G - (int)nl * GPC;
-              if (2 * gi + w < a.LWs) word = let[(size_t)nl * a.LWs + 2 * gi + w];
+              if (2 * gi + w < g.LWs()) word = let[(size_t)nl * g.LWs() + 2 * gi + w];
             }
-            vcount += stats_window_piece<NPW>(reinterpret_cast<unsigned short*>(swin), lane, word, G < ngl, gi, GPC, a.Lv);
+            vcount += stats_window_piece<NPW>(reinterpret_cast<unsigned short*>(swin), lane, word, G < ngl, gi, GPC, g.Lv());
           }
           __builtin_amdgcn_wave_barrier();
           {
@@ -1421,12 +1464,12 @@
             if (valid) {
               nl = fastdiv_tile((uint32_t)G, a.sg.divGPC);
               s = 32 * (G - (int)nl * GPC) + (lane & 31);
-              valid = s < a.Lf;
+              valid = s < g.Lf();
             }
             float* col = sPt + lane;
             if (valid) {
               const uint32_t gn = a.rng.seq_offset + (uint32_t)(n0 + nl);
-              const LetterWin<M> win = letter_window<M>(let + (size_t)nl * a.LWs, s);
+              const LetterWin<M> win = letter_window<M>(let + (size_t)nl * g.LWs(), s);
 #pragma unroll
               for (int strand = 0; strand <= C::DS; ++strand) {
                 float x[KP], p[KP];
@@ -1438,10 +1481,10 @@
                 uint32_t* dst = (strand ? a.hmp : a.hm) + (size_t)(n0 + nl) * per + (size_t)s * NW;
 #pragma unroll
                 for (int w = 0; w < NW; ++w) {
-                  if (!(a.debug & 4)) store1_streaming(dst + w, mask[w]);
+                  if (!(dbg & 4)) store1_streaming(dst + w, mask[w]);
                   nset += __popc(mask[w]);
                 }
-                if constexpr (DEFER) nset += (int)defer_units(pend, nl * (uint32_t)a.nhb + (uint32_t)s, (uint32_t)strand, st, true);
+                if constexpr (DEFER) nset += (int)defer_units(pend, nl * (uint32_t)g.nhb() + (uint32_t)s, (uint32_t)strand, st, true);
 #pragma unroll
                 for (int k = 0; k < C::K; ++k) col[(size_t)(strand * KW + k) * STATS_RS] = p[k];
               }
@@ -1459,11 +1502,11 @@
         }
       }
       if (!fused_pass) {
-      for (uint32_t it = threadIdx.x; it < (uint32_t)(ns * a.nhb); it += blockDim.x) {
-        const uint32_t nl = fastdiv_tile(it, a.divHB);
-        const int s = (int)(it - nl * (uint32_t)a.nhb);
+      for (uint32_t it = threadIdx.x; it < (uint32_t)(ns * g.nhb()); it += TB) {
+        const uint32_t nl = g.div_hb(it);
+        const int s = (int)(it - nl * (uint32_t)g.nhb());
         const uint32_t gn = a.rng.seq_offset + (uint32_t)(n0 + nl);
-        const uint32_t* lrow = let + nl * (uint32_t)a.LWs;
+        const uint32_t* lrow = let + nl * (uint32_t)g.LWs();
         const LetterWin<M> win = letter_window<M>(lrow, s);
 #pragma unroll
         for (int strand = 0; strand <= C::DS; ++strand) {
@@ -1487,7 +1530,7 @@
             uint32_t* dst = (strand ? a.hmp : a.hm) + (size_t)n0 * per + it * (uint32_t)NW;
 #pragma unroll
             for (int w = 0; w < NW; ++w) {
-              if (!(a.debug & 4)) store1_streaming(dst + w, mask[w]);
+              if (!(dbg & 4)) store1_streaming(dst + w, mask[w]);
               nset += __popc(mask[w]);
             }
           } else {
@@ -1504,42 +1547,59 @@
       }
       if constexpr (DEFER) drain_queue(st, st == a.steps - 1);
     }
-    if (a.steps == 0) __syncthreads();
-    if (a.steps == 0 && !(a.debug & 4)) {
+    const bool round_trip = !GP::CT && a.steps == 0;
+    if (round_trip) __syncthreads();
+    if (round_trip && !(dbg & 4)) {
       const uint32_t nwords = (uint32_t)ns * per;
       const size_t g0 = (size_t)n0 * per;
       auto lds_index = [&](uint32_t i) {
-        const uint32_t nl = fastdiv_tile(i, a.divLfw);
+        const uint32_t nl = g.template div_lfw<NW>(i);
         return nl * (uint32_t)rowW + (uint32_t)((M - 1) * NW) + (i - nl * per);
       };
       if (((g0 | nwords) & 3u) == 0u) {
-        for (uint32_t i4 = threadIdx.x; i4 < nwords / 4; i4 += blockDim.x) {
+        for (uint32_t i4 = threadIdx.x; i4 < nwords / 4; i4 += TB) {
           const uint32_t d0 = lds_index(4 * i4), d1 = lds_index(4 * i4 + 1), d2 = lds_index(4 * i4 + 2), d3 = lds_index(4 * i4 + 3);
           store4_streaming(a.hm + g0 + 4 * (size_t)i4, hm[d0], hm[d1], hm[d2], hm[d3]);
           if (C::DS) store4_streaming(a.hmp + g0 + 4 * (size_t)i4, hmp[d0], hmp[d1], hmp[d2], hmp[d3]);
         }
       } else {
-        for (uint32_t i = threadIdx.x; i < nwords; i += blockDim.x) {
+        for (uint32_t i = threadIdx.x; i < nwords; i += TB) {
           const uint32_t d = lds_index(i);
           a.hm[g0 + i] = hm[d];
           if (C::DS) a.hmp[g0 + i] = hmp[d];
         }
       }
     }
-    if (a.vout && !(a.debug & 4))
-      for (int idx = threadIdx.x; idx < ns * a.LWs; idx += blockDim.x)
-        a.vout[(size_t)n0 * a.LWs + idx] = let[idx];
+    if (a.vout && !(dbg & 4))
+      for (int idx = threadIdx.x; idx < ns * g.LWs(); idx += TB)
+        a.vout[(size_t)n0 * g.LWs() + idx] = let[idx];
   }
   if (a.ones) {
     const float tot = wave_sum((float)nset);
-    if ((threadIdx.x & 63) == 0) a.ones[bid * (blockDim.x >> 6) + (threadIdx.x >> 6)] = (uint32_t)tot;
-  }
-  if (a.clock && bid == 0 && threadIdx.x == 0) {
+    if ((threadIdx.x & 63) == 0) a.ones[bid * (TB >> 6) + (threadIdx.x >> 6)] = (uint32_t)tot;
+  }
+  if constexpr (GP::PROF) {
+    if (a.clock && bid == 0 && threadIdx.x == 0) {
+      a.clock[0] += realtime_ticks() - a.clock[2];
+      a.clock[1] += shader_cycles() - a.clock[3];
+    }
+    if (a.timeline && bid == 0 && threadIdx.x == 0) a.timeline[1] = realtime_ticks();
+  }
+  if constexpr (STATS) stats_mfma_finish<C, false>(a.sg, smem, 0, bid, sacc, vcount);
+}
+
+template <class C, class GP>
+__device__ void gibbs_geo_body(const GibbsArgs& a) {
+  const bool timed = a.clock && blockIdx.x == 0 && threadIdx.x == 0;
+  if (timed) {
+    a.clock[2] = realtime_ticks();
+    a.clock[3] = shader_cycles();
+  }
+  gibbs_body<C, true, false, GP>(a);
+  if (timed) {
     a.clock[0] += realtime_ticks() - a.clock[2];
     a.clock[1] += shader_cycles() - a.clock[3];
   }
-  if (a.timeline && bid == 0 && threadIdx.x == 0) a.timeline[1] = realtime_ticks();
-  if constexpr (STATS) stats_mfma_finish<C, false>(a.sg, smem, 0, bid, sacc, vcount);
 }
 
 struct TrainLocalArgs {
@@ -1547,13 +1607,13 @@
   StatsMfmaArgs d;
 };
 
-template <class C>
+template <class C, class GP = GeomRT>
 __device__ void train_local_body(const TrainLocalArgs& a) {
   if constexpr (C::FUSE_STATS) {
     const int nG = a.g.nblocks, nD = a.d.nblocks, m = min(nG, nD), b = (int)blockIdx.x;
     const bool chain = b < 2 * m ? !(b & 1) : nG > nD;
     const int idx = b < 2 * m ? b >> 1 : b - m;
-    if (chain) gibbs_body<C, true, true>(a.g, idx);
+    if (chain) gibbs_body<C, true, true, GP>(a.g, idx);
     else stats_mfma_body<C, true, false>(a.d, idx);
   }
 }
diff --git a/crbm_amd/csrc/crbm_plan.h b/crbm_amd/csrc/crbm_plan.h
--- a/crbm_amd/csrc/crbm_plan.h
+++ b/crbm_amd/csrc/crbm_plan.h
@@ -131,6 +131,24 @@
 
 struct ChainGeom { GibbsLayout gl = {}; int threads = 0, grid = 0; bool on() const { return threads > 0; } };
 
+struct GeoSpec {
+  GibbsLayout gl = {};
+  int threads = 0, grid = 0, nchains = 0, group = 0;
+  bool aligned = false;
+  bool on() const { return threads > 0; }
+  bool serves(const GibbsLayout& l, int threads_, int grid_, int nchains_) const {
+    return on() && l.S == gl.S && l.Lv == gl.Lv && l.nvb == gl.nvb && l.nhb == gl.nhb && l.Lrow == gl.Lrow && l.LWs == gl.LWs &&
+           threads_ == threads && grid_ == grid && nchains_ == nchains;
+  }
+};
+inline GeoSpec geo_spec(const GibbsLayout& gl, int threads, int grid, int nchains, int NW, int group) {
+  GeoSpec s;
+  if (threads <= 0 || threads % 64 || gl.S < 1 || nchains < gl.S || nchains % gl.S || grid < 1 || grid > nchains / gl.S) return s;
+  s.gl = gl; s.threads = threads; s.grid = grid; s.nchains = nchains; s.group = group;
+  s.aligned = ((long)gl.S * gl.nhb * NW) % 4 == 0;
+  return s;
+}
+
 struct LaunchPlan {
   bool big = false;
   int G = 0, GS = 0;
@@ -141,6 +159,7 @@
   ChainGeom part;
   int chain_parts = 1, part_chains = 0;
   int gibbs_wpe = 0, gibbs_tb = 256;
+  GeoSpec geo_plain, geo_fused;
   int slab_K = 0, slab_G = 0;
   ModelShape slab_ms = {};
   const char* slab_note = nullptr;
@@ -195,6 +214,16 @@
   int threads = 0;
   for (const ChainGeom* g : {&p.chain[0], &p.chain[1], &p.solo, &p.part}) threads = std::max(threads, g->threads);
   p.gibbs_tb = gibbs_block_bound(threads);
+  const int geo_mode = env_int("CRBM_GEOM", 1);
+  if (geo_mode > 0 && !p.refusal) {
+    auto spec = [&](const ChainGeom& g, int nchains, int group) {
+      GeoSpec s = g.on() ? geo_spec(g.gl, g.threads, g.grid, nchains, p.ms.NW, group) : GeoSpec();
+      if (geo_mode == 1 && s.on() && nchains / s.gl.S < num_cu) s = GeoSpec();
+      return s;
+    };
+    p.geo_plain = p.chain_parts > 1 ? spec(p.part, p.part_chains, p.G) : spec(plain_geom(p, 1, false), B, p.GS);
+    if (p.ms.FUSE_STATS) p.geo_fused = spec(p.chain[1], B, p.G);
+  }
   return p;
 }
 
diff --git a/include/crbm_amd.h b/include/crbm_amd.h
--- a/include/crbm_amd.h
+++ b/include/crbm_amd.h
@@ -154,6 +154,7 @@
 int crbm_get_launch_info(const crbm_handle* h, crbm_launch_info* out);
 int crbm_copy_bandwidth(crbm_handle* h, int64_t bytes, int32_t reps, float* gb_per_s);
 int crbm_last_shader_clock(crbm_handle* h, float* mhz);
+int crbm_geometry_launches(const crbm_handle* h, int64_t* compiled_in, int64_t* run_time);
 int64_t crbm_gibbs_state_bytes(const crbm_handle* h);
 
 #ifdef __cplusplus
```

Result: faster. 64370 8192-chain batch Gibbs steps/s (summed over GPUs), median of 6 (+10.5%).
